# zhaowenlan1779/hekaton-system

Hardware: AMD Instinct MI355X
Metric: subcircuit Groth16 proofs/sec (whole node), big-merkle (higher is better)
Workload: dtype u32 limbs (Montgomery mod-p integers)

## Files before the change

### hekaton_system_amd/csrc/curve_ops_impl.cuh

```cuda
#pragma once
#include "msm_driver.cuh"
#include "endo.cuh"

namespace hk {

inline u32 msm_pick_c_plain(size_t n, u32 fr_bits) {
    u32 best = 4;
    double best_cost = 1e300;
    for (u32 c = 3; c <= 12; c++) {
        u32 W = (fr_bits + 2 + c - 1) / c;
        u64 NB = (u64)W << (c - 1);
        if (NB > (u64)MSM_LDS_COUNTERS) continue;
        double cost = (double)n * W + 4.0 * (double)NB;
        if (cost < best_cost) { best_cost = cost; best = c; }
    }
    return best;
}
inline u32 msm_pick_c_tables(size_t n, u32 fr_bits) {
    u32 best = 6;
    double best_cost = 1e300;
    for (u32 c = 5; c <= 16; c++) {
        u32 W = (fr_bits + 2 + c - 1) / c;
        double cost = (double)n * W + 6.0 * (double)(1u << (c - 1));
        if (cost < best_cost) { best_cost = cost; best = c; }
    }
    return best;
}

template <class C>
struct Ops final : CurveOps {
    typedef typename C::Fr Fr;
    typedef typename C::Fq Fq;
    typedef typename C::Fq2 Fq2;
    typedef VerifyRun<typename Fq::Params> Verify;
    typedef CodecRun<typename Fq::Params> Codec;

    Ops() : CurveOps(sizeof(Fr), sizeof(Fq), sizeof(Affine<Fq>), sizeof(Affine<Fq2>), sizeof(Fp12<typename Fq::Params>)) {}

    template <class F>
    struct OneMsm {
        bool small;
        const MsmPlan* p;
        u32 n;
        XYZZ<F>*xy, *tab, *res;
        Affine<F>* aff;
        SortBufs sb;
        typename MsmRun<F>::Bufs rb;

        void carve(Carve& c) {
            if (small) {
                xy = c.n<XYZZ<F>>(n);
                tab = (XYZZ<F>*)c.take(endo_tab_bytes<F>(n));
            } else {
                MsmSort<Fr>::alloc(c, *p, &sb);
                MsmRun<F>::alloc(c, *p, &rb);
            }
            res = c.n<XYZZ<F>>(1);
            aff = c.n<Affine<F>>(1);
        }
        hk_status run(hipStream_t s, const Affine<F>* bases, const void* scalars, int mont, void* out, hipMemcpyKind kind,
                      hipEvent_t ev0 = nullptr, hipEvent_t ev1 = nullptr) const {
            if (small) {
                HK_TRY(MsmRun<F>::small_msm(s, bases, scalars, mont, n, tab, xy, res));
            } else {
                HK_TRY(MsmSort<Fr>::run(s, *p, (const u32*)scalars, mont, sb));
                HK_TRY(MsmRun<F>::run(s, *p, bases, n, 0, sb, rb, res, ev0, ev1));
            }
            HK_TRY(MsmRun<F>::to_affine(s, res, aff, 1));
            HK_HIP(hipMemcpyAsync(out, aff, sizeof(Affine<F>), kind, s));
            return HK_OK;
        }
    };

    template <class F>
    static hk_status msm_plain(hk_ctx* ctx, const void* bases, size_t n_bases, const void* scalars,
                               size_t n_scalars, int mont, int checked, void* out) {
        if (checked && n_bases != n_scalars) return HK_ERR_LEN;
        size_t n = n_bases < n_scalars ? n_bases : n_scalars;
        if (n == 0) { memset(out, 0, sizeof(Affine<F>)); return HK_OK; }
        if (!bases || !scalars) return HK_ERR_ARG;
        if (n >= (1u << 26)) return HK_ERR_ARG;
        Staged in[2] = {staged(scalars, n * sizeof(Fr)), staged(bases, n * sizeof(Affine<F>))};
        LaneGuard g(ctx);
        Lane* L = g.lane;
        if (!L) return HK_ERR_DEVICE;
        const bool small = n * EndoOf<F>::K <= SPLIT_MAX_LANES && !getenv("HK_MSM_NO_SMALL");
        MsmPlan p;
        if (!small)
            p = msm_make_plan((u32)n, C::FR_BITS, msm_pick_c_plain(n, C::FR_BITS), 0xffffffffu, ctx->max_lanes0, C::Fr::Params::MOD,
                              C::Fr::Params::N);
        OneMsm<F> msm{small, &p, (u32)n};
        HK_TRY(L->carve([&](Carve& c) { stage_carve(c, in, 2); msm.carve(c); }));
        HK_TRY(stage_upload(L, in, 2));
        HK_TRY(msm.run(L->stream, (const Affine<F>*)in[1].p, in[0].p, mont, out, hipMemcpyDeviceToHost));
        return L->settle();
    }

    hk_status msm(hk_ctx* ctx, int group, const void* bases, size_t n_bases, const void* scalars,
                  size_t n_scalars, int mont, int checked, void* out) override {
        if (group == 1) return msm_plain<Fq>(ctx, bases, n_bases, scalars, n_scalars, mont, checked, out);
        return msm_plain<Fq2>(ctx, bases, n_bases, scalars, n_scalars, mont, checked, out);
    }

    size_t max_private_bytes() override {
        size_t m = MsmRun<Fq>::max_private_bytes();
        size_t b = MsmRun<Fq2>::max_private_bytes();
        if (b > m) m = b;
        b = PairRun<typename Fq::Params>::max_private_bytes();
        if (b > m) m = b;
        b = Verify::max_private_bytes();
        if (b > m) m = b;
        b = Codec::max_private_bytes();
        if (b > m) m = b;
        b = finish_private_bytes();
        return b > m ? b : m;
    }

    hk_status ntt(hk_ctx*, void*, unsigned, int, int) override;
    hk_status witness_map(hk_ctx*, const hk_csr*, const hk_csr*, const hk_csr*, size_t, size_t,
                          const void*, size_t, void*, size_t, size_t*) override;
    void ctx_release(hk_ctx*) override;
    hk_status pk_upload(hk_ctx*, const hk_pk_desc*, hk_pk**) override;
    void pk_free(hk_pk*) override;
    hk_status bases_upload(hk_ctx*, int, const void*, size_t, hk_bases**) override;
    void bases_free(hk_bases*) override;
    hk_status msm_bases(hk_ctx*, const hk_bases*, const void*, size_t, int, int, void*) override;
    hk_status fixed_base(hk_ctx*, int, const void*, const void*, size_t, int, void*) override;
    hk_status scalar_pairing(hk_ctx*, int, const void*, const void*, size_t, void*) override;
    hk_status points_lincomb(hk_ctx*, int, const void* const*, const void*, size_t, size_t, void*) override;
    template <class F>
    static hk_status points_fold(hk_ctx*, size_t, const void* const*, const void* const*, const void*, unsigned, size_t, void* const*);
    hk_status points_fold_many(hk_ctx*, int, size_t, const void* const*, const void* const*, const void*, unsigned, size_t,
                               void* const*) override;
    hk_status field_convert(hk_ctx*, int, const void*, void*, size_t, int) override;
    hk_status assignment_from_bits(hk_ctx*, const void*, size_t, const uint32_t*, const void*, size_t, void*) override;
    hk_status wprog_upload(hk_ctx*, const uint32_t*, size_t, const uint32_t*, size_t, const uint32_t*, size_t, size_t,
                           size_t, hk_wprog**) override;
    void wprog_free(hk_wprog*) override;
    hk_status wprog_run(hk_ctx*, const hk_wprog*, const uint32_t*, size_t, const uint32_t*, const void*, size_t, void*) override;
    hk_status assignment_scatter(hk_ctx*, const uint32_t*, const void*, size_t, size_t, size_t, void*) override;
    hk_status poseidon_path(hk_ctx*, const void*, size_t, const hk_poseidon_desc*, const hk_poseidon_desc*, const void*,
                            const void*, const uint32_t*, size_t, size_t, size_t, size_t, void*) override;
    hk_status pairing_products(hk_ctx*, const void* const*, size_t, const void* const*, size_t, size_t, void*) override;
    hk_status pairing_pairs(hk_ctx*, const void* const*, size_t, const void* const*, size_t, const uint32_t*, const uint32_t*, size_t,
                            size_t, void*) override;
    hk_status gt_pow(hk_ctx*, const void*, const void*, size_t, void*, int, size_t) override;
    hk_status commit(hk_ctx*, const hk_pk*, size_t, const void*, size_t, const void*, void*) override;
    hk_status commit_batch(hk_ctx*, const hk_pk*, size_t, const void*, size_t, const void*, size_t, void*) override;
    hk_status prove_batch(hk_ctx*, const hk_pk*, size_t, size_t, const ProveRow*, size_t) override;
    static size_t finish_private_bytes();
    hk_status vk_prepare(hk_ctx* ctx, const hk_vk_desc* d, hk_vk** out) override { return Verify::vk_prepare(ctx, d, out); }
    void vk_free(hk_vk* vk) override { Verify::vk_free(vk); }
    hk_status vk_alpha_beta(const hk_vk* vk, void* out) override { return Verify::vk_alpha_beta(vk, out); }
    hk_status verify_batch(hk_ctx* ctx, const hk_vk* vk, const void* a, const void* b, const void* c, const void* ds,
                           const void* inputs, size_t n, unsigned flags, const void* rand, unsigned char* verdicts) override {
        return Verify::verify_batch(ctx, vk, a, b, c, ds, inputs, n, flags, rand, verdicts);
    }
    hk_status points_check(hk_ctx* ctx, int group, const void* pts, size_t n, unsigned char* ok) override {
        return Verify::points_check(ctx, group, pts, n, ok);
    }
    hk_status qap_eval(hk_ctx*, const hk_csr*, const hk_csr*, const hk_csr*, size_t, size_t, size_t, const void*, void*,
                       void*, void*, void*, size_t*) override;
    hk_status keygen(hk_ctx*, const hk_keygen_desc*, const hk_keygen_out*, size_t*) override;
    hk_status exec_tree(hk_ctx*, const hk_exec_tree_desc*, const hk_exec_tree_out*) override;
    hk_status stage1_witness(hk_ctx*, const hk_stage1_desc*, const uint32_t*, size_t, size_t, void*) override;
    hk_status trace_sort(hk_ctx*, uint32_t, const void*, size_t, void*, uint32_t*) override;
    hk_status stage0_witness(hk_ctx*, const uint32_t*, uint32_t, uint32_t, const void*, const void*, const uint32_t*, size_t,
                             void*) override;
    hk_status r1cs_check(hk_ctx*, const hk_csr*, const hk_csr*, const hk_csr*, const void*, size_t, size_t, hk_r1cs_verdict*,
                         uint32_t*, void*, size_t) override;
    hk_status pk_r1cs_check(hk_ctx*, const hk_pk*, const void*, size_t, size_t, hk_r1cs_verdict*, uint32_t*, void*, size_t) override;
    hk_status sha_tree(hk_ctx*, const void*, uint32_t, uint32_t, uint32_t, const hk_sha_tree_out*) override;
    hk_status sha_tree_inputs(hk_ctx*, const void*, const void*, uint32_t, uint32_t, const uint32_t*, size_t, uint32_t*) override;
    hk_status ram_stage0_witness(hk_ctx*, const uint32_t*, uint32_t, uint32_t, const void*, const void*, const uint32_t*, size_t,
                                 void*) override;
    hk_status ram_stage1_witness(hk_ctx*, const hk_ram_stage1_desc*, const uint32_t*, size_t, size_t, void*) override;
    hk_status r1cs_job_trace(hk_ctx*, const hk_r1cs_job_desc*, void*) override;
    hk_status r1cs_job_witness(hk_ctx*, const hk_r1cs_job_desc*, const uint32_t*, size_t, size_t, size_t, void*) override;
    hk_status vkd_trace(hk_ctx*, const hk_vkd_desc*, void*, void*) override;
    hk_status vkd_witness(hk_ctx*, const hk_vkd_desc*, const uint32_t*, size_t, size_t, const hk_vkd_cols*, void*) override;
    hk_status vkd_tree(hk_ctx*, const hk_vkd_tree_desc*, void*, void*, uint8_t*) override;
    hk_status scalar_powers(hk_ctx*, const void*, size_t, size_t, void*) override;
    hk_status ipa_quotient(hk_ctx*, const void*, size_t, const void*, const void*, size_t, void*) override;
    hk_status class_power_sums(hk_ctx*, const void*, const uint32_t*, size_t, size_t, void*) override;
    hk_status field_sqrt(hk_ctx* ctx, int which, const void* in, size_t n, void* out, unsigned char* ok) override {
        return Codec::field_sqrt(ctx, which, in, n, out, ok);
    }
    hk_status points_decompress(hk_ctx* ctx, int group, const void* x_canon, const unsigned char* flags, size_t n, int check,
                                void* points_out, unsigned char* status) override {
        return Codec::points_decompress(ctx, group, x_canon, flags, n, check, points_out, status);
    }
    hk_status points_compress(hk_ctx* ctx, int group, const void* points, size_t n, void* x_canon_out,
                              unsigned char* flags_out) override {
        return Codec::points_compress(ctx, group, points, n, x_canon_out, flags_out);
    }
};

}
```

### hekaton_system_amd/csrc/h_basis.cuh

```cuda
#pragma once
#include "ntt_host.cuh"
#include "csr.cuh"
#include "endo.cuh"
#include "h_basis_plan.h"

namespace hk {

template <class Fr, class F>
__device__ XYZZ<F> hb_mul(const XYZZ<F>& p, const Fr& s_mont, const EndoSplit<2>& E) {
    XYZZ<F> acc = XYZZ<F>::inf();
    if (p.is_inf()) return acc;
    Fr k = Fr::from_mont(s_mont);
    u32 c[8], mag[2][6];
    HK_UNROLL for (int l = 0; l < 8; l++) c[l] = l < Fr::N ? k.v[l] : 0u;
    u32 neg = endo_decompose<2>(c, E, mag);
    XYZZ<F> t[3];
    Affine<F> q;
    q.x = p.x; q.y = p.y;
    t[0] = p;
    t[1] = p;
    t[1].x = EndoOf<F>::apply(q).x;
    if (neg & 1u) t[0].y = F::neg(p.y);
    if (neg & 2u) t[1].y = F::neg(p.y);
    t[2] = ec_add_ni(t[0], t[1]);
    HK_NOUNROLL for (int b = EndoOf<F>::STEPS - 1; b >= 0; b--) {
        u32 m = ((mag[0][b >> 5] >> (b & 31)) & 1u) | (((mag[1][b >> 5] >> (b & 31)) & 1u) << 1);
        if (m == 0 && acc.is_inf()) continue;
        acc = ec_dbl_ni(acc);
        if (m) acc = ec_add_ni(acc, t[m - 1]);
    }
    return acc;
}

template <class Fr, class F>
__global__ void __launch_bounds__(64)
k_hb_load(const Affine<F>* __restrict__ h_g, u32 h_len, u32 log_m, const Fr* __restrict__ pw_ginv, Fr c0, Fr c1,
          EndoSplit<2> E, XYZZ<F>* __restrict__ x) {
    u32 i = blockIdx.x * blockDim.x + threadIdx.x;
    if (i >> log_m) return;
    const u32 v = blockIdx.y;
    u32 r = log_m ? (__brev(i) >> (32 - log_m)) : 0u;
    XYZZ<F> o = XYZZ<F>::inf();
    if (i < h_len) {
        Fr s = v ? c1 : Fr::mul(c0, pow_from_tables(pw_ginv, i, log_m));
        o = hb_mul(XYZZ<F>::from_affine(ld_vec(&h_g[i])), s, E);
    }
    st_vec(&x[((size_t)v << log_m) + r], o);
}

template <class Fr, class F>
__global__ void __launch_bounds__(64)
k_hb_stage(XYZZ<F>* __restrict__ x, const Fr* __restrict__ tws, u32 s, u32 log_m, EndoSplit<2> E) {
    u32 t = blockIdx.x * blockDim.x + threadIdx.x;
    if (t >> (log_m - 1)) return;
    XYZZ<F>* vec = x + ((size_t)blockIdx.y << log_m);
    const u32 half = 1u << s, pos = t & (half - 1u);
    const size_t i0 = ((size_t)(t >> s) << (s + 1)) | pos, i1 = i0 + half;
    XYZZ<F> u = ld_vec(&vec[i0]), w = ld_vec(&vec[i1]);
    if (pos) w = hb_mul(w, fr_load(&tws[(half - 1u) + pos]), E);
    st_vec(&vec[i0], ec_add_ni(u, w));
    st_vec(&vec[i1], ec_add_ni(u, ec_neg(w)));
}

template <class Fr, class F>
__global__ void __launch_bounds__(64)
k_hb_ccols(const u64* __restrict__ col_ptr, const u32* __restrict__ row, const u32* __restrict__ src,
           const Fr* __restrict__ val, const Affine<F>* __restrict__ g, const u32* __restrict__ hv,
           const Affine<F>* __restrict__ heavy, const Affine<F>* __restrict__ ck_last, u32 first_last, u32 n_v,
           EndoSplit<2> E, XYZZ<F>* __restrict__ out) {
    u32 k = blockIdx.x * blockDim.x + threadIdx.x;
    if (k >= n_v) return;
    XYZZ<F> acc = XYZZ<F>::inf();
    if (hv[k]) {
        acc = XYZZ<F>::from_affine(ld_vec(&heavy[hv[k] - 1]));
    } else {
        HK_NOUNROLL for (u64 e = col_ptr[k]; e < col_ptr[k + 1]; e++)
            acc = ec_add_ni(acc, hb_mul(XYZZ<F>::from_affine(ld_vec(&g[row[e]])), fr_load(&val[src[e]]), E));
    }
    acc = ec_neg(acc);
    if (k >= first_last) acc = ec_madd_ni(acc, ld_vec(&ck_last[k - first_last]));
    st_vec(&out[k], acc);
}

template <class C>
struct HBasis {
    typedef typename C::Fr Fr;
    typedef typename C::Fq Fq;
    typedef NttHost<C> N;

    static size_t private_bytes() {
        size_t m = 0;
        for (const void* k : {(const void*)k_hb_load<Fr, Fq>, (const void*)k_hb_stage<Fr, Fq>, (const void*)k_hb_ccols<Fr, Fq>}) {
            size_t b = hk_private_bytes_of(k);
            if (b > m) m = b;
        }
        return m;
    }

    static hk_status transform(hk_ctx* ctx, NttTables* T, const Affine<Fq>* h_g, u32 h_len, u32 log_m, Affine<Fq>* hat,
                               Affine<Fq>* g) {
        const size_t m = (size_t)1 << log_m;
        LaneGuard lg(ctx);
        Lane* L = lg.lane;
        if (!L) return HK_ERR_DEVICE;
        XYZZ<Fq>* x;
        Fq* pref;
        HK_TRY(L->carve([&](Carve& c) { x = c.n<XYZZ<Fq>>(2 * m); pref = c.n<Fq>(2 * m); }));
        hipStream_t s = L->stream;
        static const EndoSplit<2> E = EndoOf<Fq>::split();
        Fr minv = N::size_inv(log_m), zinv = N::vanishing_inv_on_coset(log_m);
        Fr c1 = Fr::mul(zinv, minv), c0 = Fr::mul(c1, Fr::mul(minv, minv));
        hipLaunchKernelGGL((k_hb_load<Fr, Fq>), dim3((u32)((m + 63) / 64), 2), dim3(64), 0, s, h_g, h_len, log_m,
                           (const Fr*)T->pw_ginv, c0, c1, E, x);
        for (u32 st = 0; st < log_m; st++)
            hipLaunchKernelGGL((k_hb_stage<Fr, Fq>), dim3((u32)((m / 2 + 63) / 64), 2), dim3(64), 0, s, x, (const Fr*)T->tw_inv,
                               st, log_m, E);
        HK_HIP(hipGetLastError());
        HK_TRY(MsmRun<Fq>::batch_affine(s, x, hat, pref, (u32)m));
        HK_TRY(MsmRun<Fq>::batch_affine(s, x + m, g, pref + m, (u32)m));
        return L->settle();
    }

    static hk_status c_columns(hk_ctx* ctx, const CsrDev& Cm, size_t n_v, u32 log_m, const Affine<Fq>* g, const void* ck_last,
                               size_t n1, Affine<Fq>* out) {
        const size_t m = (size_t)1 << log_m, nnz = Cm.nnz;
        std::vector<u64> rp(Cm.n_rows + 1), col_ptr;
        std::vector<u32> cl(nnz), row, src;
        HK_HIP(hipMemcpy(rp.data(), Cm.row_ptr, 8 * rp.size(), hipMemcpyDeviceToHost));
        if (nnz) HK_HIP(hipMemcpy(cl.data(), Cm.col, 4 * nnz, hipMemcpyDeviceToHost));
        if (Cm.n_rows > m || !hb_transpose(rp.data(), cl.data(), Cm.n_rows, n_v, col_ptr, row, src)) return HK_ERR_ARG;
        const u32 thr = hb_heavy_threshold(getenv("HK_H_BASIS_HEAVY_COL"));
        std::vector<u32> hv(n_v, 0);
        std::vector<Affine<Fq>> heavy;
        for (size_t k = 0; k < n_v; k++)
            if (hb_col_is_heavy(col_ptr[k + 1] - col_ptr[k], thr)) hv[k] = 1;
        if (std::find(hv.begin(), hv.end(), 1u) != hv.end()) {
            std::vector<Fr> vals(nnz), dense(m, Fr::zero());
            HK_HIP(hipMemcpy(vals.data(), Cm.val, sizeof(Fr) * nnz, hipMemcpyDeviceToHost));
            hk_bases* bh = nullptr;
            HK_TRY(ctx->ops->bases_upload(ctx, 1, g, m, &bh));
            hk_status st = HK_OK;
            for (size_t k = 0; k < n_v && st == HK_OK; k++) {
                if (!hv[k]) continue;
                for (u64 e = col_ptr[k]; e < col_ptr[k + 1]; e++) dense[row[e]] = Fr::add(dense[row[e]], vals[src[e]]);
                Affine<Fq> pt;
                st = ctx->ops->msm_bases(ctx, bh, dense.data(), m, 1, 1, &pt);
                for (u64 e = col_ptr[k]; e < col_ptr[k + 1]; e++) dense[row[e]] = Fr::zero();
                heavy.push_back(pt);
                hv[k] = (u32)heavy.size();
            }
            ctx->ops->bases_free(bh);
            HK_TRY(st);
        }
        Staged in[6] = {staged(col_ptr.data(), 8 * col_ptr.size()), staged(row.data(), 4 * nnz), staged(src.data(), 4 * nnz),
                        staged(hv.data(), 4 * n_v), staged(heavy.data(), sizeof(Affine<Fq>) * heavy.size()),
                        staged(n1 ? ck_last : nullptr, sizeof(Affine<Fq>) * n1)};
        LaneGuard lg(ctx);
        Lane* L = lg.lane;
        if (!L) return HK_ERR_DEVICE;
        XYZZ<Fq>* xy;
        Fq* pref;
        HK_TRY(L->carve([&](Carve& c) { stage_carve(c, in, 6); xy = c.n<XYZZ<Fq>>(n_v); pref = c.n<Fq>(n_v); }));
        HK_TRY(stage_upload(L, in, 6));
        static const EndoSplit<2> E = EndoOf<Fq>::split();
        hipLaunchKernelGGL((k_hb_ccols<Fr, Fq>), dim3((u32)((n_v + 63) / 64)), dim3(64), 0, L->stream, (const u64*)in[0].p,
                           (const u32*)in[1].p, (const u32*)in[2].p, (const Fr*)Cm.val, g, (const u32*)in[3].p,
                           (const Affine<Fq>*)in[4].p, (const Affine<Fq>*)in[5].p, (u32)(n_v - n1), (u32)n_v, E, xy);
        HK_HIP(hipGetLastError());
        HK_TRY(MsmRun<Fq>::batch_affine(L->stream, xy, out, pref, (u32)n_v));
        return L->settle();
    }
};

}
```

### hekaton_system_amd/csrc/hk_core.hip

```cpp
#include <utility>
#include "hk_internal.h"
#include "job_args.h"
#include <hsa/hsa.h>
#include <hsa/hsa_ext_amd.h>
#include <atomic>

namespace hk {

static hsa_status_t scratch_limit_cb(hsa_agent_t a, void* data) {
    hsa_device_type_t type;
    if (hsa_agent_get_info(a, HSA_AGENT_INFO_DEVICE, &type) != HSA_STATUS_SUCCESS || type != HSA_DEVICE_TYPE_GPU)
        return HSA_STATUS_SUCCESS;
    uint64_t mx = 0;
    if (hsa_agent_get_info(a, (hsa_agent_info_t)HSA_AMD_AGENT_INFO_SCRATCH_LIMIT_MAX, &mx) == HSA_STATUS_SUCCESS && mx) {
        uint64_t* best = (uint64_t*)data;
        if (*best == 0 || mx < *best) *best = mx;
    }
    return HSA_STATUS_SUCCESS;
}
static uint64_t scratch_limit_bytes() {
    static const uint64_t v = [] {
        uint64_t best = 0;
        if (hsa_init() == HSA_STATUS_SUCCESS) {
            (void)hsa_iterate_agents(scratch_limit_cb, &best);
// ... 458 lines not shown
    return ctx->ops->pairing_products(ctx, lhs_g1, n_lhs, rhs_g2, n_rhs, n, gt_out);
}
hk_status hk_multi_pairing(hk_ctx* ctx, const void* g1, const void* g2, size_t n, void* gt_out) {
    if (!ctx || !gt_out || (n && (!g1 || !g2))) return HK_ERR_ARG;
    const void* l[1] = {n ? g1 : (const void*)gt_out};
    const void* r[1] = {n ? g2 : (const void*)gt_out};
    return ctx->ops->pairing_products(ctx, l, 1, r, 1, n, gt_out);
}
hk_status hk_vk_prepare(hk_ctx* ctx, const hk_vk_desc* desc, hk_vk** out) {
    if (!ctx || !desc || !out) return HK_ERR_ARG;
    return ctx->ops->vk_prepare(ctx, desc, out);
}
void hk_vk_free(hk_vk* vk) {
    if (vk) vk->ops->vk_free(vk);
}
hk_status hk_vk_alpha_beta(const hk_vk* vk, void* gt_out) {
    if (!vk || !gt_out) return HK_ERR_ARG;
    return vk->ops->vk_alpha_beta(vk, gt_out);
}
hk_status hk_verify_batch(hk_ctx* ctx, const hk_vk* vk, const void* a_g1, const void* b_g2, const void* c_g1, const void* ds_g1,
                          const void* inputs_mont, size_t n, unsigned flags, const void* rand_mont, uint8_t* verdicts) {
    if (!ctx || !vk || vk->ctx != ctx) return HK_ERR_ARG;
    return ctx->ops->verify_batch(ctx, vk, a_g1, b_g2, c_g1, ds_g1, inputs_mont, n, flags, rand_mont, verdicts);
}
hk_status hk_points_check_g1(hk_ctx* ctx, const void* points, size_t n, uint8_t* ok) {
    if (!ctx || (n && (!points || !ok))) return HK_ERR_ARG;
    return ctx->ops->points_check(ctx, 1, points, n, ok);
}
hk_status hk_points_check_g2(hk_ctx* ctx, const void* points, size_t n, uint8_t* ok) {
    if (!ctx || (n && (!points || !ok))) return HK_ERR_ARG;
    return ctx->ops->points_check(ctx, 2, points, n, ok);
}
hk_status hk_ctx_gt_bytes(const hk_ctx* ctx, size_t* gt) {
    if (!ctx || !gt) return HK_ERR_ARG;
    *gt = ctx->ops->gt_bytes;
    return HK_OK;
}
hk_status hk_field_convert(hk_ctx* ctx, int which, const void* in, void* out, size_t n, int to_mont) {
    if (!ctx || (which != 0 && which != 1) || (n && (!in || !out))) return HK_ERR_ARG;
    return ctx->ops->field_convert(ctx, which, in, out, n, to_mont);
}
hk_status hk_ntt(hk_ctx* ctx, void* data, unsigned log_m, int inverse, int coset) {
    if (!ctx || !data) return HK_ERR_ARG;
    return ctx->ops->ntt(ctx, data, log_m, inverse, coset);
}
hk_status hk_witness_map(hk_ctx* ctx, const hk_csr* A, const hk_csr* B, const hk_csr* C, size_t n_inst,
                         size_t n_constraints, const void* z_mont, size_t n_v, void* h_out,
                         size_t h_capacity, size_t* m_out) {
    if (!ctx || !A || !B || !C || !z_mont || !h_out) return HK_ERR_ARG;
    return ctx->ops->witness_map(ctx, A, B, C, n_inst, n_constraints, z_mont, n_v, h_out, h_capacity, m_out);
}
hk_status hk_pk_upload(hk_ctx* ctx, const hk_pk_desc* desc, hk_pk** out) {
    if (!ctx || !desc || !out) return HK_ERR_ARG;
    return ctx->ops->pk_upload(ctx, desc, out);
}
void hk_pk_free(hk_pk* pk) {
    if (!pk) return;
    pk->ops->pk_free(pk);
}
hk_status hk_commit(hk_ctx* ctx, const hk_pk* pk, size_t stage, const void* w, size_t n, const void* kappa,
                    void* out) {
    if (!ctx || !pk || !kappa || !out) return HK_ERR_ARG;
    return ctx->ops->commit(ctx, pk, stage, w, n, kappa, out);
}
hk_status hk_commit_batch(hk_ctx* ctx, const hk_pk* pk, size_t stage, const void* w, size_t n, const void* kappas, size_t batch,
                          void* out) {
    if (!ctx || !pk || (batch && (!kappas || !out))) return HK_ERR_ARG;
    return ctx->ops->commit_batch(ctx, pk, stage, w, n, kappas, batch, out);
}
hk_status hk_prove(hk_ctx* ctx, const hk_pk* pk, const void* z, size_t n_v, const void* r, const void* s,
                   const void* kappas, size_t n_kappas, void* a, void* b, void* c) {
    if (!ctx || !pk || !z || !r || !s || !a || !b || !c) return HK_ERR_ARG;
    HK_TRY(ctx->ops->prove_batch(ctx, pk, n_v, n_kappas, nullptr, 0));
    if (n_kappas && !kappas) return HK_ERR_ARG;
    const hk::ProveCall call = {{z, r, s, kappas, a, b, c}, n_v, n_kappas};
    if (hk::gather_trace() && hk::tl_prev_chunk_end_us)
        fprintf(stderr, "[hekaton] gather arrive gap_us=%lld\n", (long long)(hk::now_us() - hk::tl_prev_chunk_end_us));
    hk::ProveResult res = ctx->prove_q.submit(pk, call, [&](const hk_pk* key, hk::ProveCoalescer::Member* const* ms, size_t n) {
        std::vector<hk::ProveRow> rows(n);
        for (size_t i = 0; i < n; i++) rows[i] = ms[i]->item->row;
        hk_status st = ctx->ops->prove_batch(ctx, key, ms[0]->item->n_v, ms[0]->item->n_kappas, rows.data(), n);
        hk_timings t = tl_last_timings;
        const float f = 1.0f / (float)n;
        for (float* x : {&t.total_ms, &t.digits_ms, &t.msm_a_ms, &t.msm_b_g1_ms, &t.msm_b_g2_ms, &t.msm_l_ms, &t.witness_map_ms,
                         &t.msm_h_ms, &t.finish_ms, &t.accum_kernel_ms, &t.accum_h_ms, &t.keygen_qap_ms, &t.keygen_scalars_ms,
                         &t.keygen_sweeps_ms})
            *x *= f;
        if (t.accum_kernel_launches) t.accum_kernel_launches = 4;
        t.batch_proofs = (uint32_t)n;
        int64_t end_us = 0;
        if (hk::gather_trace()) {
            end_us = hk::now_us();
            fprintf(stderr, "[hekaton] gather chunk n=%zu arena_allocs=%u\n", n, hk::g_arena_allocs.load());
        }
        for (size_t i = 0; i < n; i++) ms[i]->result = hk::ProveResult{st, t, end_us};
    });
    hk::tl_prev_chunk_end_us = res.end_us;
    tl_last_timings = res.timings;
    return res.status;
}
hk_status hk_prove_batch(hk_ctx* ctx, const hk_pk* pk, const void* z, size_t n_v, const void* r, const void* s,
                         const void* kappas, size_t n_kappas, size_t batch, void* a, void* b, void* c) {
    if (!ctx || !pk) return HK_ERR_ARG;
    HK_TRY(ctx->ops->prove_batch(ctx, pk, n_v, n_kappas, nullptr, 0));
    if (batch == 0) return HK_OK;
    if (!z || !r || !s || !a || !b || !c || (n_kappas && !kappas)) return HK_ERR_ARG;
    const size_t fr = ctx->ops->fr_bytes, g1 = ctx->ops->g1_bytes, g2 = ctx->ops->g2_bytes;
    std::vector<hk::ProveRow> rows(batch);
    for (size_t i = 0; i < batch; i++)
        rows[i] = {(const char*)z + i * n_v * fr, (const char*)r + i * fr, (const char*)s + i * fr,
                   n_kappas ? (const char*)kappas + i * n_kappas * fr : nullptr, (char*)a + i * g1, (char*)b + i * g2,
                   (char*)c + i * g1};
    return ctx->ops->prove_batch(ctx, pk, n_v, n_kappas, rows.data(), batch);
}

hk_status hk_qap_eval(hk_ctx* ctx, const hk_csr* A, const hk_csr* B, const hk_csr* C, size_t n_inst, size_t n_constraints,
                      size_t n_v, const void* t, void* a, void* b, void* c, void* zt, size_t* m_out) {
    if (!ctx) return HK_ERR_ARG;
    return ctx->ops->qap_eval(ctx, A, B, C, n_inst, n_constraints, n_v, t, a, b, c, zt, m_out);
}
hk_status hk_keygen(hk_ctx* ctx, const hk_keygen_desc* desc, const hk_keygen_out* out, size_t* m_out) {
    if (!ctx || !desc || !out) return HK_ERR_ARG;
    return ctx->ops->keygen(ctx, desc, out, m_out);
}
hk_status hk_exec_tree(hk_ctx* ctx, const hk_exec_tree_desc* desc, const hk_exec_tree_out* out) {
    if (!ctx || !desc || !out) return HK_ERR_ARG;
    return ctx->ops->exec_tree(ctx, desc, out);
}
hk_status hk_stage1_witness(hk_ctx* ctx, const hk_stage1_desc* desc, const uint32_t* sub_index, size_t batch, size_t n_v,
                            void* z_out) {
    if (!ctx || !desc) return HK_ERR_ARG;
    return ctx->ops->stage1_witness(ctx, desc, sub_index, batch, n_v, z_out);
}
hk_status hk_trace_sort(hk_ctx* ctx, uint32_t entry_fields, const void* time_entries_mont, size_t n_entries,
                        void* addr_entries_mont_out, uint32_t* perm_out) {
    if (!ctx) return HK_ERR_ARG;
    return ctx->ops->trace_sort(ctx, entry_fields, time_entries_mont, n_entries, addr_entries_mont_out, perm_out);
}
hk_status hk_stage0_witness(hk_ctx* ctx, const uint32_t* offsets, uint32_t n_sub, uint32_t n_portals, const void* time_entries_mont,
                            const void* addr_entries_mont, const uint32_t* sub_index, size_t batch, void* w_out) {
    if (!ctx) return HK_ERR_ARG;
    return ctx->ops->stage0_witness(ctx, offsets, n_sub, n_portals, time_entries_mont, addr_entries_mont, sub_index, batch, w_out);
}
hk_status hk_r1cs_check(hk_ctx* ctx, const hk_csr* A, const hk_csr* B, const hk_csr* C, const void* z_mont, size_t n_v, size_t batch,
                        hk_r1cs_verdict* verdicts, uint32_t* bad_rows, void* bad_vals, size_t cap) {
    if (!ctx || !A || !B || !C) return HK_ERR_ARG;
    return ctx->ops->r1cs_check(ctx, A, B, C, z_mont, n_v, batch, verdicts, bad_rows, bad_vals, cap);
}
hk_status hk_pk_r1cs_check(hk_ctx* ctx, const hk_pk* pk, const void* z_mont, size_t n_v, size_t batch, hk_r1cs_verdict* verdicts,
                           uint32_t* bad_rows, void* bad_vals, size_t cap) {
    if (!ctx || !pk) return HK_ERR_ARG;
    return ctx->ops->pk_r1cs_check(ctx, pk, z_mont, n_v, batch, verdicts, bad_rows, bad_vals, cap);
}
hk_status hk_sha_tree(hk_ctx* ctx, const void* leaves, uint32_t n_sub, uint32_t ns, uint32_t n_portals, const hk_sha_tree_out* out) {
    if (!ctx || !leaves || !out) return HK_ERR_ARG;
    return ctx->ops->sha_tree(ctx, leaves, n_sub, ns, n_portals, out);
}
hk_status hk_sha_tree_inputs(hk_ctx* ctx, const void* leaves, const void* digests, uint32_t n_sub, uint32_t n_inputs,
                             const uint32_t* sub_index, size_t batch, uint32_t* inputs_out) {
    if (!ctx) return HK_ERR_ARG;
    return ctx->ops->sha_tree_inputs(ctx, leaves, digests, n_sub, n_inputs, sub_index, batch, inputs_out);
}
hk_status hk_ram_stage0_witness(hk_ctx* ctx, const uint32_t* offsets, uint32_t n_sub, uint32_t n_portals,
                                const void* time_entries_mont, const void* addr_entries_mont, const uint32_t* sub_index, size_t batch,
                                void* w_out) {
    if (!ctx) return HK_ERR_ARG;
    return ctx->ops->ram_stage0_witness(ctx, offsets, n_sub, n_portals, time_entries_mont, addr_entries_mont, sub_index, batch, w_out);
}
hk_status hk_ram_stage1_witness(hk_ctx* ctx, const hk_ram_stage1_desc* desc, const uint32_t* sub_index, size_t batch, size_t n_v,
                                void* z_out) {
    if (!ctx || !desc) return HK_ERR_ARG;
    return ctx->ops->ram_stage1_witness(ctx, desc, sub_index, batch, n_v, z_out);
}
hk_status hk_r1cs_job_trace(hk_ctx* ctx, const hk_r1cs_job_desc* desc, void* time_entries_mont_out) {
    if (!ctx || !desc) return HK_ERR_ARG;
    return ctx->ops->r1cs_job_trace(ctx, desc, time_entries_mont_out);
}
hk_status hk_r1cs_job_witness(hk_ctx* ctx, const hk_r1cs_job_desc* desc, const uint32_t* sub_index, size_t batch, size_t n_v,
                              size_t body_col0, void* z_out) {
    if (!ctx || !desc) return HK_ERR_ARG;
    return ctx->ops->r1cs_job_witness(ctx, desc, sub_index, batch, n_v, body_col0, z_out);
}
hk_status hk_vkd_trace(hk_ctx* ctx, const hk_vkd_desc* desc, void* values_mont_out, void* time_entries_mont_out) {
    if (!ctx || !desc) return HK_ERR_ARG;
    return ctx->ops->vkd_trace(ctx, desc, values_mont_out, time_entries_mont_out);
}
hk_status hk_vkd_witness(hk_ctx* ctx, const hk_vkd_desc* desc, const uint32_t* sub_index, size_t batch, size_t n_v,
                         const hk_vkd_cols* cols, void* z_out) {
    if (!ctx || !desc) return HK_ERR_ARG;
    return ctx->ops->vkd_witness(ctx, desc, sub_index, batch, n_v, cols, z_out);
}
hk_status hk_vkd_tree(hk_ctx* ctx, const hk_vkd_tree_desc* desc, void* siblings_mont_out, void* roots_mont_out, uint8_t* status_out) {
    if (!ctx || !desc) return HK_ERR_ARG;
    return ctx->ops->vkd_tree(ctx, desc, siblings_mont_out, roots_mont_out, status_out);
}
hk_status hk_scalar_powers(hk_ctx* ctx, const void* x_mont, size_t n, size_t reps, void* out) {
    if (!ctx) return HK_ERR_ARG;
    return ctx->ops->scalar_powers(ctx, x_mont, n, reps, out);
}
hk_status hk_ipa_quotient(hk_ctx* ctx, const void* challenges_mont, size_t l, const void* rho_mont, const void* z_mont,
                          size_t shift, void* q_out) {
    if (!ctx) return HK_ERR_ARG;
    return ctx->ops->ipa_quotient(ctx, challenges_mont, l, rho_mont, z_mont, shift, q_out);
}
hk_status hk_class_power_sums(hk_ctx* ctx, const void* x_mont, const uint32_t* class_of, size_t n, size_t n_classes,
                              void* sums_out) {
    if (!ctx) return HK_ERR_ARG;
    return ctx->ops->class_power_sums(ctx, x_mont, class_of, n, n_classes, sums_out);
}

static bool codec_bufs_bad(const void* const* in, const size_t* in_len, int n_in, const void* const* out, const size_t* out_len,
                           int n_out) {
    for (int a = 0; a < n_in; a++)
        if (!in[a]) return true;
    for (int b = 0; b < n_out; b++) {
        if (!out[b]) return true;
        for (int a = 0; a < n_in; a++)
            if (hk::bufs_overlap(in[a], in_len[a], out[b], out_len[b])) return true;
        for (int c = 0; c < b; c++)
            if (hk::bufs_overlap(out[c], out_len[c], out[b], out_len[b])) return true;
    }
    return false;
}
hk_status hk_field_sqrt(hk_ctx* ctx, int which, const void* in_mont, size_t n, void* out_mont, uint8_t* ok) {
    if (!ctx || (which != 1 && which != 2) || n >= ((size_t)1 << 31)) return HK_ERR_ARG;
    if (n == 0) return HK_OK;
    const size_t eb = ctx->ops->fq_bytes * (size_t)which;
    const void* in[1] = {in_mont};
    const void* out[2] = {out_mont, ok};
    const size_t il[1] = {n * eb}, ol[2] = {n * eb, n};
    if (codec_bufs_bad(in, il, 1, out, ol, 2)) return HK_ERR_ARG;
    return ctx->ops->field_sqrt(ctx, which, in_mont, n, out_mont, ok);
}
static hk_status points_decompress(hk_ctx* ctx, int group, const void* x_canon, const uint8_t* flags, size_t n, int check,
                                   void* points_out, uint8_t* status) {
    if (!ctx || n >= ((size_t)1 << 31)) return HK_ERR_ARG;
    if (n == 0) return HK_OK;
    const size_t xb = ctx->ops->fq_bytes * (size_t)group;
    const void* in[2] = {x_canon, flags};
    const void* out[2] = {points_out, status};
    const size_t il[2] = {n * xb, n}, ol[2] = {2 * n * xb, n};
    if (codec_bufs_bad(in, il, 2, out, ol, 2)) return HK_ERR_ARG;
    return ctx->ops->points_decompress(ctx, group, x_canon, flags, n, check, points_out, status);
}
static hk_status points_compress(hk_ctx* ctx, int group, const void* points, size_t n, void* x_canon_out, uint8_t* flags_out) {
    if (!ctx || n >= ((size_t)1 << 31)) return HK_ERR_ARG;
    if (n == 0) return HK_OK;
    const size_t xb = ctx->ops->fq_bytes * (size_t)group;
    const void* in[1] = {points};
    const void* out[2] = {x_canon_out, flags_out};
    const size_t il[1] = {2 * n * xb}, ol[2] = {n * xb, n};
    if (codec_bufs_bad(in, il, 1, out, ol, 2)) return HK_ERR_ARG;
    return ctx->ops->points_compress(ctx, group, points, n, x_canon_out, flags_out);
}
hk_status hk_points_decompress_g1(hk_ctx* ctx, const void* x_canon, const uint8_t* flags, size_t n, int check, void* points_out,
                                  uint8_t* status) {
    return points_decompress(ctx, 1, x_canon, flags, n, check, points_out, status);
}
hk_status hk_points_decompress_g2(hk_ctx* ctx, const void* x_canon, const uint8_t* flags, size_t n, int check, void* points_out,
                                  uint8_t* status) {
    return points_decompress(ctx, 2, x_canon, flags, n, check, points_out, status);
}
hk_status hk_points_compress_g1(hk_ctx* ctx, const void* points, size_t n, void* x_canon_out, uint8_t* flags_out) {
    return points_compress(ctx, 1, points, n, x_canon_out, flags_out);
}
hk_status hk_points_compress_g2(hk_ctx* ctx, const void* points, size_t n, void* x_canon_out, uint8_t* flags_out) {
    return points_compress(ctx, 2, points, n, x_canon_out, flags_out);
}

}

extern "C" void hk_keccak_f1600(uint64_t* st) {
    static const uint64_t RC[24] = {
        0x0000000000000001ull, 0x0000000000008082ull, 0x800000000000808aull, 0x8000000080008000ull, 0x000000000000808bull,
        0x0000000080000001ull, 0x8000000080008081ull, 0x8000000000008009ull, 0x000000000000008aull, 0x0000000000000088ull,
        0x0000000080008009ull, 0x000000008000000aull, 0x000000008000808bull, 0x800000000000008bull, 0x8000000000008089ull,
        0x8000000000008003ull, 0x8000000000008002ull, 0x8000000000000080ull, 0x000000000000800aull, 0x800000008000000aull,
        0x8000000080008081ull, 0x8000000000008080ull, 0x0000000080000001ull, 0x8000000080008008ull};
    static const int ROT[5][5] = {{0, 36, 3, 41, 18}, {1, 44, 10, 45, 2}, {62, 6, 43, 15, 61}, {28, 55, 25, 21, 56}, {27, 20, 39, 8, 14}};
    auto rol = [](uint64_t x, int n) { return n ? (x << n) | (x >> (64 - n)) : x; };
    for (int rnd = 0; rnd < 24; rnd++) {
        uint64_t c[5], d[5], b[25];
        for (int x = 0; x < 5; x++) c[x] = st[x] ^ st[x + 5] ^ st[x + 10] ^ st[x + 15] ^ st[x + 20];
        for (int x = 0; x < 5; x++) d[x] = c[(x + 4) % 5] ^ rol(c[(x + 1) % 5], 1);
        for (int i = 0; i < 25; i++) st[i] ^= d[i % 5];
        for (int x = 0; x < 5; x++)
            for (int y = 0; y < 5; y++) b[y + 5 * ((2 * x + 3 * y) % 5)] = rol(st[x + 5 * y], ROT[x][y]);
        for (int y = 0; y < 5; y++)
            for (int x = 0; x < 5; x++) st[x + 5 * y] = b[x + 5 * y] ^ (~b[(x + 1) % 5 + 5 * y] & b[(x + 2) % 5 + 5 * y]);
        st[0] ^= RC[rnd];
    }
}
```

### hekaton_system_amd/csrc/hk_internal.h

```cpp
#pragma once
#include <hip/hip_runtime.h>
#include <condition_variable>
#include <cstdio>
#include <cstring>
#include <map>
#include <mutex>
#include <string>
#include <vector>

#include "../../include/hekaton.h"
#include "coalesce.h"
#include "msm.cuh"
#include "stream_plan.h"

#define HK_HIP(expr)                                                                         \
    do {                                                                                     \
        hipError_t _e = (expr);                                                              \
        if (_e != hipSuccess) {                                                              \
            fprintf(stderr, "[hekaton] HIP error %s at %s:%d: %s\n", hipGetErrorName(_e),    \
                    __FILE__, __LINE__, #expr);                                              \
            return HK_ERR_DEVICE;                                                            \
        }                                                                                    \
    } while (0)

#define HK_TRY(expr)                       \
    do {                                   \
        hk_status _s = (expr);             \
        if (_s != HK_OK) return _s;        \
    } while (0)

namespace hk {

struct CurveBn254 {
    typedef Fp<Bn254FrP> Fr;
    typedef Fp<Bn254FqP> Fq;
    typedef Fp2<Bn254FqP> Fq2;
    static constexpr u32 FR_BITS = HK_BN254_FR_BITS;
    static constexpr u32 TWO_ADICITY = HK_BN254_TWO_ADICITY;
    static constexpr u32 ROOT[8] = HK_BN254_FR_ROOT;
    static constexpr u32 GEN[8] = HK_BN254_FR_GEN;
    static constexpr u32 GEN_INV[8] = HK_BN254_FR_GEN_INV;
};
struct CurveBls381 {
    typedef Fp<Bls381FrP> Fr;
    typedef Fp<Bls381FqP> Fq;
    typedef Fp2<Bls381FqP> Fq2;
    static constexpr u32 FR_BITS = HK_BLS12_381_FR_BITS;
    static constexpr u32 TWO_ADICITY = HK_BLS12_381_TWO_ADICITY;
    static constexpr u32 ROOT[8] = HK_BLS12_381_FR_ROOT;
    static constexpr u32 GEN[8] = HK_BLS12_381_FR_GEN;
    static constexpr u32 GEN_INV[8] = HK_BLS12_381_FR_GEN_INV;
};

template <class F> struct ScalarOf;
template <> struct ScalarOf<CurveBn254::Fq> { typedef CurveBn254::Fr type; };
template <> struct ScalarOf<CurveBn254::Fq2> { typedef CurveBn254::Fr type; };
template <> struct ScalarOf<CurveBls381::Fq> { typedef CurveBls381::Fr type; };
template <> struct ScalarOf<CurveBls381::Fq2> { typedef CurveBls381::Fr type; };

struct Carve {
    char* base = nullptr;
    size_t off = 0;
    void* take(size_t bytes) {
        size_t o = (off + 255) & ~(size_t)255;
        off = o + bytes;
        return base ? base + o : nullptr;
    }
    template <class T> T* n(size_t count) { return (T*)take(count * sizeof(T)); }
};

struct Lane {
    hipStream_t stream = nullptr;
    char* arena = nullptr;
    size_t arena_cap = 0;
    hipEvent_t ev[32];
    hipStream_t side[PROVE_MAX_STREAMS - 1] = {};
    unsigned n_streams = 1;
    bool prove = false;
    bool busy = false;
    bool settled = false;
    hk_timings timings;
    std::vector<void*> retired;
    hk_ctx* owner = nullptr;

    hk_status reserve(size_t bytes);
    template <class Fn> hk_status carve(Fn&& fn) {
        Carve count;
        fn(count);
        HK_TRY(reserve(count.off));
        Carve real;
        real.base = arena;
        fn(real);
        if (real.off != count.off) {
            fprintf(stderr, "[hekaton] scratch carve is not deterministic (%zu bytes counted, %zu carved)\n", count.off, real.off);
            return HK_ERR_DEVICE;
        }
        settled = false;
        return HK_OK;
    }
    hipStream_t stream_at(unsigned i) const { return i ? side[i - 1] : stream; }
    hk_status settle() {
        for (unsigned i = 0; i < n_streams; i++) HK_HIP(hipStreamSynchronize(stream_at(i)));
        settled = true;
        return HK_OK;
    }
};

struct NttTables;

struct ProveRow {
    const void* z;
    const void* r;
    const void* s;
    const void* kappas;
    void *a, *b, *c;
};

struct ProveResult {
    hk_status status;
    hk_timings timings;
    int64_t end_us;
};

enum { PROVE_GATHER_US = 1000 };

struct ProveCall {
    ProveRow row;
    size_t n_v, n_kappas;
};

enum { PROVE_COALESCE_RUNNING = 2 };
typedef Coalescer<const hk_pk*, ProveCall, ProveResult> ProveCoalescer;

}

namespace hk {
struct CurveOps {
    const size_t fr_bytes, fq_bytes, g1_bytes, g2_bytes, gt_bytes;

    virtual hk_status msm(hk_ctx*, int group, const void* bases, size_t n_bases, const void* scalars,
                          size_t n_scalars, int mont, int checked, void* out) = 0;
    virtual size_t max_private_bytes() = 0;
    virtual hk_status ntt(hk_ctx*, void* data, unsigned log_m, int inverse, int coset) = 0;
    virtual hk_status witness_map(hk_ctx*, const hk_csr* A, const hk_csr* B, const hk_csr* C, size_t n_inst,
                                  size_t n_c, const void* z, size_t n_v, void* h_out, size_t h_cap, size_t* m_out) = 0;
    virtual void ctx_release(hk_ctx*) = 0;
    virtual hk_status pk_upload(hk_ctx*, const hk_pk_desc*, hk_pk**) = 0;
    virtual void pk_free(hk_pk*) = 0;
    virtual hk_status bases_upload(hk_ctx*, int group, const void* bases, size_t n, hk_bases** out) = 0;
    virtual void bases_free(hk_bases*) = 0;
    virtual hk_status msm_bases(hk_ctx*, const hk_bases*, const void* scalars, size_t n_scalars, int mont, int checked,
                                void* out) = 0;
    virtual hk_status fixed_base(hk_ctx*, int group, const void* base, const void* scalars, size_t n, int mont,
                                 void* out) = 0;
    virtual hk_status scalar_pairing(hk_ctx*, int group, const void* points, const void* scalars, size_t n, void* out) = 0;
    virtual hk_status points_lincomb(hk_ctx*, int group, const void* const* vecs, const void* coeffs, size_t k, size_t n,
                                     void* out) = 0;
    virtual hk_status points_fold_many(hk_ctx*, int group, size_t k, const void* const* lo, const void* const* hi,
                                       const void* coeffs, unsigned neg_mask, size_t n, void* const* out) = 0;
    virtual hk_status field_convert(hk_ctx*, int which, const void* in, void* out, size_t n, int to_mont) = 0;
    virtual hk_status assignment_from_bits(hk_ctx*, const void* bits, size_t n_v, const uint32_t* full_cols,
                                           const void* full_vals, size_t n_full, void* z_out) = 0;
    virtual hk_status wprog_upload(hk_ctx*, const uint32_t* ops, size_t n_ops, const uint32_t* refs, size_t n_refs,
                                   const uint32_t* map, size_t n_v, size_t n_values, size_t n_inputs, hk_wprog** out) = 0;
    virtual void wprog_free(hk_wprog*) = 0;
    virtual hk_status wprog_run(hk_ctx*, const hk_wprog*, const uint32_t* inputs, size_t batch, const uint32_t* full_cols,
                                const void* full_vals, size_t n_full, void* z_out) = 0;
    virtual hk_status assignment_scatter(hk_ctx*, const uint32_t* full_cols, const void* full_vals, size_t n_full, size_t batch,
                                         size_t n_v, void* z_out) = 0;
    virtual hk_status poseidon_path(hk_ctx*, const void* consts, size_t n_consts, const hk_poseidon_desc* leaf_hash,
                                    const hk_poseidon_desc* node_hash, const void* leaf, const void* siblings,
                                    const uint32_t* index, size_t depth, size_t batch, size_t n_v, size_t col0, void* z_out) = 0;
    virtual hk_status pairing_products(hk_ctx*, const void* const* lhs, size_t n_lhs, const void* const* rhs, size_t n_rhs,
                                       size_t n, void* out) = 0;
    virtual hk_status pairing_pairs(hk_ctx*, const void* const* lhs, size_t n_lhs, const void* const* rhs, size_t n_rhs,
                                    const uint32_t* pair_lhs, const uint32_t* pair_rhs, size_t n_pairs, size_t n, void* out) = 0;
    virtual hk_status gt_pow(hk_ctx*, const void* gt_in, const void* scalars, size_t n, void* gt_out, int in_gt,
                             size_t group_len) = 0;
    virtual hk_status commit(hk_ctx*, const hk_pk*, size_t stage, const void* w, size_t n, const void* kappa,
                             void* out) = 0;
    virtual hk_status commit_batch(hk_ctx*, const hk_pk*, size_t stage, const void* w, size_t n, const void* kappas, size_t batch,
                                   void* out) = 0;
    virtual hk_status prove_batch(hk_ctx*, const hk_pk*, size_t n_v, size_t n_kappas, const ProveRow* rows, size_t batch) = 0;
    virtual hk_status vk_prepare(hk_ctx*, const hk_vk_desc*, hk_vk**) = 0;
    virtual void vk_free(hk_vk*) = 0;
    virtual hk_status vk_alpha_beta(const hk_vk*, void*) = 0;
    virtual hk_status verify_batch(hk_ctx*, const hk_vk*, const void* a, const void* b, const void* c, const void* ds,
                                   const void* inputs, size_t n, unsigned flags, const void* rand, unsigned char* verdicts) = 0;
    virtual hk_status points_check(hk_ctx*, int group, const void* pts, size_t n, unsigned char* ok) = 0;
    virtual hk_status qap_eval(hk_ctx*, const hk_csr* A, const hk_csr* B, const hk_csr* C, size_t n_inst, size_t n_c, size_t n_v,
                               const void* t, void* a, void* b, void* c, void* zt, size_t* m_out) = 0;
    virtual hk_status keygen(hk_ctx*, const hk_keygen_desc*, const hk_keygen_out*, size_t* m_out) = 0;
    virtual hk_status exec_tree(hk_ctx*, const hk_exec_tree_desc*, const hk_exec_tree_out*) = 0;
    virtual hk_status stage1_witness(hk_ctx*, const hk_stage1_desc*, const uint32_t* sub_index, size_t batch, size_t n_v,
                                     void* z_out) = 0;
    virtual hk_status trace_sort(hk_ctx*, uint32_t entry_fields, const void* time_entries, size_t n_entries, void* addr_entries_out,
                                 uint32_t* perm_out) = 0;
    virtual hk_status stage0_witness(hk_ctx*, const uint32_t* offsets, uint32_t n_sub, uint32_t n_portals, const void* time_entries,
                                     const void* addr_entries, const uint32_t* sub_index, size_t batch, void* w_out) = 0;
    virtual hk_status r1cs_check(hk_ctx*, const hk_csr* A, const hk_csr* B, const hk_csr* C, const void* z, size_t n_v, size_t batch,
                                 hk_r1cs_verdict* verdicts, uint32_t* bad_rows, void* bad_vals, size_t cap) = 0;
    virtual hk_status pk_r1cs_check(hk_ctx*, const hk_pk*, const void* z, size_t n_v, size_t batch, hk_r1cs_verdict* verdicts,
                                    uint32_t* bad_rows, void* bad_vals, size_t cap) = 0;
    virtual hk_status sha_tree(hk_ctx*, const void* leaves, uint32_t n_sub, uint32_t ns, uint32_t n_portals,
                               const hk_sha_tree_out* out) = 0;
    virtual hk_status sha_tree_inputs(hk_ctx*, const void* leaves, const void* digests, uint32_t n_sub, uint32_t n_inputs,
                                      const uint32_t* sub_index, size_t batch, uint32_t* inputs_out) = 0;

    virtual hk_status ram_stage0_witness(hk_ctx*, const uint32_t* offsets, uint32_t n_sub, uint32_t n_portals,
                                         const void* time_entries, const void* addr_entries, const uint32_t* sub_index,
                                         size_t batch, void* w_out) = 0;
    virtual hk_status ram_stage1_witness(hk_ctx*, const hk_ram_stage1_desc*, const uint32_t* sub_index, size_t batch, size_t n_v,
                                         void* z_out) = 0;
    virtual hk_status r1cs_job_trace(hk_ctx*, const hk_r1cs_job_desc*, void* time_entries_out) = 0;
    virtual hk_status r1cs_job_witness(hk_ctx*, const hk_r1cs_job_desc*, const uint32_t* sub_index, size_t batch, size_t n_v,
                                       size_t body_col0, void* z_out) = 0;
    virtual hk_status vkd_trace(hk_ctx*, const hk_vkd_desc*, void* values_out, void* time_entries_out) = 0;
    virtual hk_status vkd_witness(hk_ctx*, const hk_vkd_desc*, const uint32_t* sub_index, size_t batch, size_t n_v,
                                  const hk_vkd_cols* cols, void* z_out) = 0;
    virtual hk_status vkd_tree(hk_ctx*, const hk_vkd_tree_desc*, void* siblings_out, void* roots_out, uint8_t* status_out) = 0;
    virtual hk_status scalar_powers(hk_ctx*, const void* x, size_t n, size_t reps, void* out) = 0;
    virtual hk_status ipa_quotient(hk_ctx*, const void* challenges, size_t l, const void* rho, const void* z, size_t shift,
                                   void* q_out) = 0;
    virtual hk_status class_power_sums(hk_ctx*, const void* x, const uint32_t* class_of, size_t n, size_t n_classes,
                                       void* sums_out) = 0;
    virtual hk_status field_sqrt(hk_ctx*, int which, const void* in, size_t n, void* out, unsigned char* ok) = 0;
    virtual hk_status points_decompress(hk_ctx*, int group, const void* x_canon, const unsigned char* flags, size_t n, int check,
                                        void* points_out, unsigned char* status) = 0;
    virtual hk_status points_compress(hk_ctx*, int group, const void* points, size_t n, void* x_canon_out,
                                      unsigned char* flags_out) = 0;

protected:
    CurveOps(size_t fr, size_t fq, size_t g1, size_t g2, size_t gt)
        : fr_bytes(fr), fq_bytes(fq), g1_bytes(g1), g2_bytes(g2), gt_bytes(gt) {}
    ~CurveOps() = default;
};
CurveOps* curve_ops_bn254();
CurveOps* curve_ops_bls381();
}

struct hk_ctx {
    hk_curve curve;
    hk::CurveOps* ops = nullptr;
    int device;
    int profiling = 0;
    std::mutex mu;
    std::condition_variable cv;
    std::vector<hk::Lane*> lanes;
    size_t max_lanes = 8;
    std::vector<hk::Lane*> prove_lanes;
    unsigned prove_streams = 1;
    std::condition_variable prove_cv;
    hk::NttTables* ntt = nullptr;
    hk_timings last;
    uint32_t max_lanes0 = 262144;
    void* presize_kernel = nullptr;
    struct FbTable { int group; std::string base; void* table; bool ready; };
    enum { FB_CACHE_MAX = 8 };
    std::vector<FbTable> fb_cache;
    hk::ProveCoalescer prove_q;
    explicit hk_ctx(long gather_us)
        : prove_q(hk::PROVE_COALESCE_RUNNING, HK_PROVE_BATCH_CHUNK, hk::ProveResult{HK_ERR_NOMEM, {}, 0}, gather_us) {}
};

struct hk_pk {
    hk::CurveOps* ops;
    hk_ctx* ctx;
    void* impl;
};

struct hk_vk {
    hk::CurveOps* ops;
    hk_ctx* ctx;
    void* impl;
};

struct hk_bases {
    hk::CurveOps* ops;
    hk_ctx* ctx;
    void* impl;
};

namespace hk {
struct WprogImpl {
    uint32_t *ops = nullptr, *refs = nullptr, *map = nullptr;
    uint32_t n_ops = 0, n_refs = 0, n_values = 0, n_inputs = 0;
    size_t n_v = 0;
};
}
struct hk_wprog {
    hk::CurveOps* ops;
    hk_ctx* ctx;
    hk::WprogImpl* impl;
};

namespace hk {

struct ProveLaneTag {};
struct LaneGuard {
    hk_ctx* ctx;
    Lane* lane;
    LaneGuard(hk_ctx* c);
    LaneGuard(hk_ctx* c, ProveLaneTag);
    ~LaneGuard();
};

bool is_device_ptr(const void* p);
static inline hipMemcpyKind h2d_kind(const void* src) {
    return is_device_ptr(src) ? hipMemcpyDeviceToDevice : hipMemcpyHostToDevice;
}
static inline float ev_ms(hipEvent_t a, hipEvent_t b) {
    float ms = 0.f;
    if (hipEventElapsedTime(&ms, a, b) != hipSuccess) { (void)hipGetLastError(); return 0.f; }
    return ms;
}

struct Staged {
    const void* buf;
    size_t bytes;
    size_t scratch;
    void* p;
};
static inline Staged staged(const void* buf, size_t bytes) {
    return {buf, bytes, buf && !is_device_ptr(buf) ? bytes : 0, nullptr};
}
static inline void stage_carve(Carve& c, Staged* s, size_t n) {
    for (size_t k = 0; k < n; k++) {
        void* slice = c.take(s[k].scratch);
        s[k].p = s[k].scratch ? slice : (void*)s[k].buf;
    }
}
static inline hk_status stage_upload(Lane* L, const Staged* s, size_t n) {
    for (size_t k = 0; k < n; k++)
        if (s[k].scratch) HK_HIP(hipMemcpyAsync(s[k].p, s[k].buf, s[k].bytes, hipMemcpyHostToDevice, L->stream));
    return HK_OK;
}
static inline hk_status stage_download(Lane* L, const Staged* s, size_t n) {
    for (size_t k = 0; k < n; k++)
        if (s[k].scratch) HK_HIP(hipMemcpyAsync((void*)s[k].buf, s[k].p, s[k].bytes, hipMemcpyDeviceToHost, L->stream));
    return HK_OK;
}

}
```

### hekaton_system_amd/csrc/msm.cuh

```cuda
#pragma once
#include <cstdlib>
#include "ec.cuh"

namespace hk {

constexpr int MSM_MAX_LEVELS = 16;
#ifndef HK_MSM_LVL_L
#define HK_MSM_LVL_L 16
#endif
constexpr u32 MSM_LVL_L = HK_MSM_LVL_L;
constexpr int MSM_TAIL_THREADS = 256;
constexpr int MSM_WSUM_THREADS = 256;
#ifndef HK_MSM_SORT_THREADS
#define HK_MSM_SORT_THREADS 1024
#endif
constexpr int MSM_SORT_THREADS = HK_MSM_SORT_THREADS;
constexpr int MSM_ENTRY_GROUP_SHIFT = 26;
constexpr int MSM_LDS_COUNTERS = 32768;
constexpr u32 MSM_RANK_NONE = 0xffffffffu;

struct MsmPlan {
    u32 n;
    u32 c;
    u32 B;
    u32 W;
    u32 WP;
    u32 F;
    u32 NB;
    u32 n_levels;
    u32 T[MSM_MAX_LEVELS];
    u32 Lmin0;
    u32 gshift;
    u32 chunk;
    u32 K;
    u32 kconst[10];
};

struct LevelInfo { u32 count, L, active; };
HK_HD LevelInfo msm_level_info(const MsmPlan& p, u32 E, int k) {
    LevelInfo li;
    li.count = E;
    u32 L = (E + p.T[0] - 1) / p.T[0];
    if (L < p.Lmin0) L = p.Lmin0;
    li.L = L;
    li.active = (E + L - 1) / L;
    for (int j = 1; j <= k; j++) {
        li.count = 2 * li.active;
        li.L = MSM_LVL_L;
        li.active = (li.count + li.L - 1) / li.L;
    }
    return li;
}

HK_HD size_t msm_sorted_stride(const MsmPlan& p) { return (size_t)p.n * p.W + 1; }
HK_HD size_t msm_digits_stride(const MsmPlan& p) { return (size_t)p.n * p.W + 8; }
HK_HD size_t msm_p1_stride(const MsmPlan& p) { return p.n_levels > 1 ? 2ull * p.T[1] : 2ull; }

#if defined(__HIPCC__)

template <class Fr>
__device__ __forceinline__ void msm_load_scalar(const u32* scalars, size_t i, int is_mont,
                                                const MsmPlan& p, u32 (&sp)[10]) {
    Fr s;
    const uint4* src = reinterpret_cast<const uint4*>(scalars + i * Fr::N);
#pragma unroll
    for (int k = 0; k < Fr::N / 4; k++) {
        uint4 v = src[k];
        s.v[4 * k] = v.x; s.v[4 * k + 1] = v.y; s.v[4 * k + 2] = v.z; s.v[4 * k + 3] = v.w;
    }
    if (is_mont) s = Fr::from_mont(s);
    u64 carry = 0;
#pragma unroll
    for (int k = 0; k < Fr::N; k++) {
        carry += (u64)s.v[k] + p.kconst[k];
        sp[k] = (u32)carry;
        carry >>= 32;
    }
    carry += p.kconst[Fr::N];
    sp[Fr::N] = (u32)carry;
    sp[Fr::N + 1] = 0;
}

template <u32 C>
__device__ __forceinline__ int msm_digit_at(const u32 (&sp)[10], u32 w) {
    const u32 o = C * w;
    const u32 limb = o >> 5, sh = o & 31;
    u32 e = sp[limb] >> sh;
    if (sh + C > 32) e |= sp[limb + 1] << (32 - sh);
    return (int)(e & ((1u << C) - 1u)) - (int)(1u << (C - 1));
}

template <class Fr, u32 C>
__device__ __forceinline__ void msm_hist_scalar(const u32 (&sp)[10], size_t i, const MsmPlan& p, short* __restrict__ digits,
                                                u32* h) {
    constexpr u32 WMAX = (Fr::N * 32 + 2 + C - 1) / C;
#pragma unroll
    for (u32 w = 0; w < WMAX; w++) {
        if (w >= p.W) break;
        int d = msm_digit_at<C>(sp, w);
        digits[(size_t)w * p.n + i] = (short)d;
        if (d != 0) {
            u32 mag = d < 0 ? (u32)(-d) : (u32)d;
            atomicAdd(&h[(p.WP == 1 ? 0u : w % p.WP) * p.B + mag - 1], 1u);
        }
    }
}

template <class Fr>
__global__ void __launch_bounds__(MSM_SORT_THREADS)
k_msm_hist(const u32* __restrict__ scalars_all, size_t scalar_stride_words, int is_mont, MsmPlan p,
           u32* __restrict__ count_all, short* __restrict__ digits_all) {
    const size_t pr = blockIdx.y;
    const u32* __restrict__ scalars = scalars_all + pr * scalar_stride_words;
    u32* __restrict__ count = count_all + pr * p.NB;
    short* __restrict__ digits = digits_all + pr * msm_digits_stride(p);
    __shared__ u32 h[MSM_LDS_COUNTERS];
    for (u32 b = threadIdx.x; b < p.NB; b += blockDim.x) h[b] = 0;
    __syncthreads();
    size_t base = (size_t)blockIdx.x * p.chunk;
    for (u32 k = threadIdx.x; k < p.chunk; k += blockDim.x) {
        size_t i = base + k;
        if (i >= p.n) break;
        u32 sp[10];
        msm_load_scalar<Fr>(scalars, i, is_mont, p, sp);
        switch (p.c) {
#define HK_HIST_C(C) case C: msm_hist_scalar<Fr, C>(sp, i, p, digits, h); break;
            HK_HIST_C(3) HK_HIST_C(4) HK_HIST_C(5) HK_HIST_C(6) HK_HIST_C(7) HK_HIST_C(8) HK_HIST_C(9) HK_HIST_C(10)
            HK_HIST_C(11) HK_HIST_C(12) HK_HIST_C(13) HK_HIST_C(14) HK_HIST_C(15) HK_HIST_C(16)
#undef HK_HIST_C
        }
    }
    __syncthreads();
    for (u32 b = threadIdx.x; b < p.NB; b += blockDim.x) {
        u32 v = h[b];
        if (v) atomicAdd(&count[b], v);
    }
}

template <int UNUSED>
__global__ void __launch_bounds__(1024)
k_msm_scan(const u32* __restrict__ count_all, u32* __restrict__ start_all, u32* __restrict__ cursor_all, u32 NB) {
    const size_t pr = blockIdx.x;
    const u32* __restrict__ count = count_all + pr * NB;
    u32* __restrict__ start = start_all + pr * (NB + 1);
    u32* __restrict__ cursor = cursor_all + pr * NB;
    __shared__ u32 part[1024];
    u32 per = (NB + 1023) / 1024;
    u32 lo = threadIdx.x * per, hi = min(lo + per, NB);
    u32 s = 0;
    for (u32 b = lo; b < hi; b++) s += count[b];
    part[threadIdx.x] = s;
    __syncthreads();
    for (u32 off = 1; off < 1024; off <<= 1) {
        u32 v = threadIdx.x >= off ? part[threadIdx.x - off] : 0;
        __syncthreads();
        part[threadIdx.x] += v;
        __syncthreads();
    }
    u32 run = threadIdx.x ? part[threadIdx.x - 1] : 0;
    for (u32 b = lo; b < hi; b++) {
        start[b] = run;
        cursor[b] = run;
        run += count[b];
    }
    if (threadIdx.x == 1023) start[NB] = part[1023];
}

__device__ __forceinline__ u32 msm_mag(int d) { return d < 0 ? (u32)(-d) : (u32)d; }
template <class Fr>
__global__ void __launch_bounds__(MSM_SORT_THREADS)
k_msm_scatter(const short* __restrict__ digits_all, MsmPlan p, u32* __restrict__ cursor_all, u32* __restrict__ sorted_all) {
    const size_t pr = blockIdx.y;
    const short* __restrict__ digits = digits_all + pr * msm_digits_stride(p);
    u32* __restrict__ cursor = cursor_all + pr * p.NB;
    u32* __restrict__ sorted = sorted_all + pr * msm_sorted_stride(p);
    __shared__ u32 h[MSM_LDS_COUNTERS];
    for (u32 b = threadIdx.x; b < p.NB; b += blockDim.x) h[b] = 0;
    __syncthreads();
    size_t base = (size_t)blockIdx.x * p.chunk;
    for (u32 k = threadIdx.x; k < p.chunk; k += blockDim.x) {
        size_t i = base + k;
        if (i >= p.n) break;
        for (u32 w = 0; w < p.W; w++) {
            int d = digits[(size_t)w * p.n + i];
            if (d != 0) atomicAdd(&h[(w % p.WP) * p.B + msm_mag(d) - 1], 1u);
        }
    }
    __syncthreads();
    for (u32 b = threadIdx.x; b < p.NB; b += blockDim.x) {
        u32 v = h[b];
        if (v) h[b] = atomicAdd(&cursor[b], v);
    }
    __syncthreads();
    for (u32 k = threadIdx.x; k < p.chunk; k += blockDim.x) {
        size_t i = base + k;
        if (i >= p.n) break;
        for (u32 w = 0; w < p.W; w++) {
            int d = digits[(size_t)w * p.n + i];
            if (d != 0) {
                u32 pos = atomicAdd(&h[(w % p.WP) * p.B + msm_mag(d) - 1], 1u);
                sorted[pos] = ((w / p.WP) << p.gshift) | (u32)i | (d < 0 ? 0x80000000u : 0u);
            }
        }
    }
}

constexpr u32 MSM_SUB_TILE = 1024;
constexpr u32 MSM_SUB_WORDS = MSM_SUB_TILE / 64;
constexpr int MSM_SUB_THREADS = 256;
HK_HD u32 msm_sub_tiles(const MsmPlan& src) { return (u32)(((u64)src.n * src.W) / MSM_SUB_TILE) + 1u; }

template <int UNUSED>
__global__ void __launch_bounds__(MSM_SUB_THREADS)
k_msm_sub_mark(const u32* __restrict__ sorted_all, const u32* __restrict__ start_all, MsmPlan ps,
               const u32* __restrict__ rank, u64* __restrict__ mask_all, u32* __restrict__ tcount_all) {
    const size_t pr = blockIdx.y;
    const u32 tiles = msm_sub_tiles(ps);
    const u32 tile = blockIdx.x * (MSM_SUB_THREADS / 64) + (threadIdx.x >> 6), lane = threadIdx.x & 63;
    if (tile >= tiles) return;
    const u32* __restrict__ sorted = sorted_all + pr * msm_sorted_stride(ps);
    const u32 E = start_all[pr * (ps.NB + 1) + ps.NB];
    u64* __restrict__ mask = mask_all + (pr * tiles + tile) * MSM_SUB_WORDS;
    const u32 imask = (1u << ps.gshift) - 1u;
    u32 kept = 0;
#pragma unroll 4
    for (u32 k = 0; k < MSM_SUB_WORDS; k++) {
        const u32 pos = tile * MSM_SUB_TILE + k * 64 + lane;
        bool keep = false;
        if (pos < E) keep = rank[sorted[pos] & imask] != MSM_RANK_NONE;
        const u64 word = __ballot(keep);
        if (lane == 0) mask[k] = word;
        kept += (u32)__popcll(word);
    }
    if (lane == 0) tcount_all[pr * tiles + tile] = kept;
}

template <int UNUSED>
__global__ void __launch_bounds__(MSM_SUB_THREADS)
k_msm_sub_emit(const u32* __restrict__ sorted_all, MsmPlan ps, const u32* __restrict__ rank,
               const u64* __restrict__ mask_all, const u32* __restrict__ toff_all, MsmPlan pd, u32* __restrict__ out_all) {
    const size_t pr = blockIdx.y;
    const u32 tiles = msm_sub_tiles(ps);
    const u32 tile = blockIdx.x * (MSM_SUB_THREADS / 64) + (threadIdx.x >> 6), lane = threadIdx.x & 63;
    if (tile >= tiles) return;
    const u32* __restrict__ sorted = sorted_all + pr * msm_sorted_stride(ps);
    u32* __restrict__ out = out_all + pr * msm_sorted_stride(pd);
    const u64* __restrict__ mask = mask_all + (pr * tiles + tile) * MSM_SUB_WORDS;
    const u32 imask = (1u << ps.gshift) - 1u;
    const u64 below = ((u64)1 << lane) - 1u;
    u32 run = toff_all[pr * tiles + tile] - toff_all[pr * tiles];
#pragma unroll 4
    for (u32 k = 0; k < MSM_SUB_WORDS; k++) {
        const u64 word = mask[k];
        if ((word >> lane) & 1u) {
            const u32 e = sorted[tile * MSM_SUB_TILE + k * 64 + lane];
            const u32 g = (e & 0x7fffffffu) >> ps.gshift;
            out[run + (u32)__popcll(word & below)] = (e & 0x80000000u) | (g << pd.gshift) | rank[e & imask];
        }
        run += (u32)__popcll(word);
    }
}

template <int UNUSED>
__global__ void __launch_bounds__(256)
k_msm_sub_starts(const u32* __restrict__ start_src_all, MsmPlan ps, const u64* __restrict__ mask_all,
                 const u32* __restrict__ toff_all, u32* __restrict__ start_dst_all) {
    const size_t pr = blockIdx.y;
    const u32 b = blockIdx.x * blockDim.x + threadIdx.x;
    if (b > ps.NB) return;
    const u32 tiles = msm_sub_tiles(ps);
    const u32 pos = start_src_all[pr * (ps.NB + 1) + b];
    const u32 tile = pos / MSM_SUB_TILE, in = pos % MSM_SUB_TILE;
    const u64* __restrict__ mask = mask_all + (pr * tiles + tile) * MSM_SUB_WORDS;
    u32 v = toff_all[pr * tiles + tile] - toff_all[pr * tiles];
    for (u32 k = 0; k < in / 64; k++) v += (u32)__popcll(mask[k]);
    if (in % 64) v += (u32)__popcll(mask[in / 64] & (((u64)1 << (in % 64)) - 1u));
    start_dst_all[pr * (ps.NB + 1) + b] = v;
}

template <class T>
__device__ __forceinline__ T ld_vec(const T* p) {
    static_assert(sizeof(T) % 16 == 0, "16-byte multiples");
    T r;
    const uint4* s = reinterpret_cast<const uint4*>(p);
    uint4* d = reinterpret_cast<uint4*>(&r);
#pragma unroll
    for (int k = 0; k < (int)(sizeof(T) / 16); k++) d[k] = s[k];
    return r;
}
// ... 455 lines not shown
```

### hekaton_system_amd/csrc/msm_driver.cuh

```cuda
#pragma once
#include "hk_internal.h"
#include "pairing.cuh"

namespace hk {

static inline size_t hk_private_bytes_of(const void* kernel) {
    hipFuncAttributes fa;
    if (hipFuncGetAttributes(&fa, kernel) != hipSuccess) { (void)hipGetLastError(); return 0; }
    return (size_t)fa.localSizeBytes;
}

struct SortBufs {
    u32* count;
    u32* start;
    u32* cursor;
    u32* sorted;
    short* digits;
    u64* mask = nullptr;
    u32* tcount = nullptr;
    u32* toff = nullptr;
    u32* tops = nullptr;
};

template <class Fr>
struct MsmSort {
    static void alloc(Carve& c, const MsmPlan& p, SortBufs* out, u32 batch = 1);
    static void alloc_sub(Carve& c, const MsmPlan& src, const MsmPlan& p, SortBufs* out, u32 batch = 1);
    static hk_status sublist(hipStream_t s, const MsmPlan& src, const SortBufs& sb_src, const MsmPlan& dst, const u32* rank,
                             const SortBufs& sb_dst, u32 batch = 1);
    static hk_status run(hipStream_t s, const MsmPlan& p, const u32* scalars_d, int is_mont,
                         const SortBufs& sb, bool count_is_zero = false, u32 batch = 1, size_t scalar_stride = 0);
};

template <class F>
struct MsmRun {
    struct Bufs {
        XYZZ<F>* buckets;
        u32* pkeys[2];
        XYZZ<F>* ppts[2];
        XYZZ<F>* red;
        XYZZ<F>* wsum;
    };
    static void alloc(Carve& c, const MsmPlan& p, Bufs* out, u32 batch = 1);
    static hk_status run(hipStream_t s, const MsmPlan& p, const Affine<F>* table, u32 n_bases, u32 idx_off,
                         const SortBufs& sb, const Bufs& b, XYZZ<F>* result_d,
                         hipEvent_t ev0, hipEvent_t ev1, u32 batch = 1, u32 res_stride = 1);
    static hk_status build_tables(hipStream_t s, Affine<F>* table, u32 n, u32 groups, u32 shift_bits);
    static hk_status to_affine(hipStream_t s, const XYZZ<F>* in, Affine<F>* out, u32 n);
    static hk_status fixed_base(hipStream_t s, const Affine<F>* base, const void* scalars, int is_mont,
                                u32 n, Affine<F>* table, XYZZ<F>* xy, F* pref, Affine<F>* out, bool build_table = true);
    static hk_status batch_affine(hipStream_t s, const XYZZ<F>* in, Affine<F>* out, F* pref, u32 n);
    static hk_status scalar_mul_each(hipStream_t s, const Affine<F>* pts, const void* scalars_mont, u32 n,
                                     XYZZ<F>* xy, F* pref, Affine<F>* out, XYZZ<F>* tab = nullptr);
    static hk_status lincomb(hipStream_t s, const Affine<F>* const* vecs, const void* coeffs_mont, u32 k, u32 n,
                             XYZZ<F>* xy, F* pref, Affine<F>* out);
    static hk_status fold_endo(hipStream_t s, u32 k, const Affine<F>* const* lo, const Affine<F>* const* hi, const void* coeffs_mont,
                               u32 neg_mask, u32 n, XYZZ<F>* tab, XYZZ<F>* xy, F* pref, Affine<F>* out, bool long_mags = false);
    static hk_status small_msm(hipStream_t s, const Affine<F>* bases, const void* scalars, int mont, u32 n, XYZZ<F>* tab,
                               XYZZ<F>* xy, XYZZ<F>* result);
    static hk_status small_msm_rows(hipStream_t s, const Affine<F>* bases, const void* scalars, u32 seg, u32 batch, XYZZ<F>* tab,
                                    XYZZ<F>* xy, XYZZ<F>* result);
    static size_t max_private_bytes();
};

constexpr int PAIR_LIST_MAX = 64;
struct PairList {
    u32 n;
    unsigned char a[PAIR_LIST_MAX], b[PAIR_LIST_MAX];
};

template <class P>
struct PairRun {
    static hk_status run(hipStream_t s, const Affine<Fp<P>>* g1, const Affine<Fp2<P>>* g2, u32 n, u32 n_l, u32 n_r,
                         Fp12<P>* miller, Fp12<P>* prod, Fp12<P>* out, const PairList* pairs = nullptr);
    static size_t scratch_bytes(u32 n, u32 count, u32 n_r);
    static size_t max_private_bytes();
    static u32 steps();
    static hk_status gt_pow(hipStream_t s, const Fp12<P>* in, const void* scalars_mont, u32 n, Fp12<P>* out, bool in_gt);
    static hk_status gt_prod(hipStream_t s, const Fp12<P>* in, u32 len, u32 groups, Fp12<P>* out);
};

template <class P>
struct VerifyRun {
    static hk_status vk_prepare(hk_ctx*, const hk_vk_desc*, hk_vk**);
    static void vk_free(hk_vk*);
    static hk_status vk_alpha_beta(const hk_vk*, void* gt_out);
    static hk_status verify_batch(hk_ctx*, const hk_vk*, const void* a, const void* b, const void* c, const void* ds,
                                  const void* inputs, size_t n, unsigned flags, const void* rand, unsigned char* verdicts);
    static hk_status points_check(hk_ctx*, int group, const void* pts, size_t n, unsigned char* ok);
    static size_t max_private_bytes();
};

template <class P>
struct CodecRun {
    static hk_status field_sqrt(hk_ctx*, int which, const void* in, size_t n, void* out, unsigned char* ok);
    static hk_status points_decompress(hk_ctx*, int group, const void* x_canon, const unsigned char* flags, size_t n, int check,
                                       void* points_out, unsigned char* status);
    static hk_status points_compress(hk_ctx*, int group, const void* points, size_t n, void* x_canon_out, unsigned char* flags_out);
    static size_t max_private_bytes();
};

}
```

### hekaton_system_amd/csrc/msm_driver_impl.cuh

```cuda
#pragma once
#include <hip/hip_ext.h>
#include "msm_driver.cuh"
#include "fixed_base.cuh"
#include "endo.cuh"
#include "scan.cuh"

namespace hk {

static inline bool hk_dbg_sync() { static const bool on = getenv("HK_DEBUG_SYNC") != nullptr; return on; }
#define HK_DBG(stream, name)                                                              \
    do {                                                                                  \
        if (hk_dbg_sync()) {                                                              \
            fprintf(stderr, "[hk] launched %s\n", name); fflush(stderr);                  \
            hipError_t _e = hipStreamSynchronize(stream);                                 \
            fprintf(stderr, "[hk] finished %s: %s\n", name, hipGetErrorName(_e)); fflush(stderr); \
        }                                                                                 \
    } while (0)

template <class Fr>
void MsmSort<Fr>::alloc(Carve& c, const MsmPlan& p, SortBufs* out, u32 batch) {
    out->count = c.n<u32>((size_t)p.NB * batch);
    out->start = c.n<u32>((size_t)(p.NB + 1) * batch);
    out->cursor = c.n<u32>((size_t)p.NB * batch);
    out->sorted = c.n<u32>(msm_sorted_stride(p) * batch);
    out->digits = c.n<short>(msm_digits_stride(p) * batch);
}

template <class Fr>
void MsmSort<Fr>::alloc_sub(Carve& c, const MsmPlan& src, const MsmPlan& p, SortBufs* out, u32 batch) {
    const size_t tiles = (size_t)msm_sub_tiles(src) * batch;
    out->count = nullptr;
    out->cursor = nullptr;
    out->digits = nullptr;
    out->start = c.n<u32>((size_t)(p.NB + 1) * batch);
    out->sorted = c.n<u32>(msm_sorted_stride(p) * batch);
    out->mask = c.n<u64>(tiles * MSM_SUB_WORDS);
    out->tcount = c.n<u32>(tiles);
    out->toff = c.n<u32>(tiles);
    out->tops = c.n<u32>(scan_u32_tops_len(tiles));
}

template <class Fr>
hk_status MsmSort<Fr>::sublist(hipStream_t s, const MsmPlan& src, const SortBufs& sb_src, const MsmPlan& dst, const u32* rank,
                               const SortBufs& sb_dst, u32 batch) {
    if (batch == 0 || batch > 65535u) return HK_ERR_ARG;
    if (dst.c != src.c || dst.W != src.W || dst.WP != src.WP || dst.NB != src.NB || dst.n > src.n) return HK_ERR_ARG;
    const u32 tiles = msm_sub_tiles(src);
    if ((u64)tiles * batch > 0xffffffffull) return HK_ERR_ARG;
    const dim3 gt((tiles + MSM_SUB_THREADS / 64 - 1) / (MSM_SUB_THREADS / 64), batch);
    hipLaunchKernelGGL((k_msm_sub_mark<0>), gt, dim3(MSM_SUB_THREADS), 0, s, (const u32*)sb_src.sorted,
                       (const u32*)sb_src.start, src, rank, sb_dst.mask, sb_dst.tcount);
    HK_DBG(s, "k_msm_sub_mark");
    HK_TRY(scan_u32(s, sb_dst.tcount, sb_dst.toff, sb_dst.tops, tiles * batch));
    hipLaunchKernelGGL((k_msm_sub_emit<0>), gt, dim3(MSM_SUB_THREADS), 0, s, (const u32*)sb_src.sorted, src, rank,
                       (const u64*)sb_dst.mask, (const u32*)sb_dst.toff, dst, sb_dst.sorted);
    HK_DBG(s, "k_msm_sub_emit");
    hipLaunchKernelGGL((k_msm_sub_starts<0>), dim3((src.NB + 1 + 255) / 256, batch), dim3(256), 0, s,
                       (const u32*)sb_src.start, src, (const u64*)sb_dst.mask, (const u32*)sb_dst.toff, sb_dst.start);
    HK_DBG(s, "k_msm_sub_starts");
    HK_HIP(hipGetLastError());
    return HK_OK;
}

template <class Fr>
hk_status MsmSort<Fr>::run(hipStream_t s, const MsmPlan& p, const u32* scalars_d, int is_mont,
                           const SortBufs& sb, bool count_is_zero, u32 batch, size_t scalar_stride) {
    if (p.NB > (u32)MSM_LDS_COUNTERS || p.c < 3 || p.c > 16) return HK_ERR_ARG;
    if (batch == 0 || batch > 65535u) return HK_ERR_ARG;
    if (!count_is_zero) HK_HIP(hipMemsetAsync(sb.count, 0, sizeof(u32) * p.NB * batch, s));
    u32 blocks = (p.n + p.chunk - 1) / p.chunk;
    if (blocks == 0) blocks = 1;
    const size_t words = scalar_stride * (sizeof(Fr) / sizeof(u32));
    hipLaunchKernelGGL((k_msm_hist<Fr>), dim3(blocks, batch), dim3(MSM_SORT_THREADS), 0, s,
                       scalars_d, words, is_mont, p, sb.count, sb.digits);
    HK_DBG(s, "k_msm_hist");
    hipLaunchKernelGGL((k_msm_scan<0>), dim3(batch), dim3(1024), 0, s, sb.count, sb.start, sb.cursor, p.NB);
    HK_DBG(s, "k_msm_scan");
    hipLaunchKernelGGL((k_msm_scatter<Fr>), dim3(blocks, batch), dim3(MSM_SORT_THREADS), 0, s,
                       (const short*)sb.digits, p, sb.cursor, sb.sorted);
    HK_DBG(s, "k_msm_scatter");
    HK_HIP(hipGetLastError());
    return HK_OK;
}

template <class F>
static inline MsmPlan msm_lane_plan(const MsmPlan& p0, u32 batch = 1) {
    MsmPlan p = p0;
    u32 lanes = (u32)AccumOcc<F>::waves * 65536u / (batch ? batch : 1u);
    msm_set_lanes(p, lanes ? lanes : 1u);
    return p;
}

template <class F>
void MsmRun<F>::alloc(Carve& c, const MsmPlan& p0, Bufs* out, u32 batch) {
    const MsmPlan p = msm_lane_plan<F>(p0, batch);
    const size_t n0 = 2ull * p.T[0], n1 = msm_p1_stride(p);
    out->buckets = c.n<XYZZ<F>>((size_t)(p.NB + 1) * batch);
    out->pkeys[0] = c.n<u32>(n0 * batch);
    out->ppts[0] = c.n<XYZZ<F>>(n0 * batch);
    out->pkeys[1] = c.n<u32>(n1 * batch);
    out->ppts[1] = c.n<XYZZ<F>>(n1 * batch);
    out->red = c.n<XYZZ<F>>((size_t)p.WP * (p.B / p.K) * batch);
    out->wsum = c.n<XYZZ<F>>((size_t)p.WP * batch);
}

template <class F>
hk_status MsmRun<F>::run(hipStream_t s, const MsmPlan& p0, const Affine<F>* table, u32 n_bases, u32 idx_off,
                         const SortBufs& sb, const Bufs& b, XYZZ<F>* result_d,
                         hipEvent_t ev0, hipEvent_t ev1, u32 batch, u32 res_stride) {
    if (batch == 0 || batch > 65535u) return HK_ERR_ARG;
    const MsmPlan p = msm_lane_plan<F>(p0, batch);
    const size_t n0 = 2ull * p.T[0], n1 = msm_p1_stride(p);
    dim3 g0((p.T[0] + 63) / 64, batch);
    if (ev0 && ev1)
        hipExtLaunchKernelGGL((k_msm_accum0<F>), g0, dim3(64), 0, s, ev0, ev1, 0,
                              table, n_bases, idx_off, sb.sorted, sb.start, p, b.buckets, b.pkeys[0], b.ppts[0]);
    else
        hipLaunchKernelGGL((k_msm_accum0<F>), g0, dim3(64), 0, s,
                           table, n_bases, idx_off, sb.sorted, sb.start, p, b.buckets, b.pkeys[0], b.ppts[0]);
    HK_DBG(s, "k_msm_accum0");
    u32 k = 1;
    for (; k < p.n_levels && p.T[k] > (u32)MSM_TAIL_THREADS; k++) {
        int in = (k - 1) & 1, out = k & 1;
        hipLaunchKernelGGL((k_msm_accum_lvl<F>), dim3((p.T[k] + 63) / 64, batch), dim3(64), 0, s,
                           (int)k, b.pkeys[in], b.ppts[in], in ? n1 : n0, sb.start, p, b.buckets, b.pkeys[out], b.ppts[out],
                           out ? n1 : n0);
        HK_DBG(s, "k_msm_accum_lvl");
    }
    if (k < p.n_levels) {
        hipLaunchKernelGGL((k_msm_accum_tail<F>), dim3(batch), dim3(MSM_TAIL_THREADS), 0, s, (int)k, b.pkeys[0], b.ppts[0],
                           b.pkeys[1], b.ppts[1], sb.start, p, b.buckets);
        HK_DBG(s, "k_msm_accum_tail");
    }
    u32 J = p.B / p.K;
    if (p.WP == 1) {
        u32 blocks = (J + MSM_REDUCE_THREADS - 1) / MSM_REDUCE_THREADS;
        hipLaunchKernelGGL((k_msm_reduce_fused<F>), dim3(blocks, batch), dim3(MSM_REDUCE_THREADS), 0, s, b.buckets, sb.start, p,
                           b.red, result_d, res_stride);
        HK_DBG(s, "k_msm_reduce_fused");
    } else {
        const size_t rs = (size_t)p.WP * J;
        for (u32 pr = 0; pr < batch; pr++) {
            const XYZZ<F>* bk = b.buckets + (size_t)pr * (p.NB + 1);
            const u32* st = sb.start + (size_t)pr * (p.NB + 1);
            hipLaunchKernelGGL((k_msm_bucket_reduce<F>), dim3((p.WP * J + 63) / 64), dim3(64), 0, s, bk, st, p, b.red + pr * rs);
            HK_DBG(s, "k_msm_bucket_reduce");
            hipLaunchKernelGGL((k_msm_window_sum<F>), dim3(p.WP), dim3(MSM_WSUM_THREADS), 0, s, b.red + pr * rs, p,
                               b.wsum + (size_t)pr * p.WP);
            HK_DBG(s, "k_msm_window_sum");
            hipLaunchKernelGGL((k_msm_final<F>), dim3(1), dim3(64), 0, s, b.wsum + (size_t)pr * p.WP, p,
                               result_d + (size_t)pr * res_stride);
            HK_DBG(s, "k_msm_final");
        }
    }
    HK_HIP(hipGetLastError());
    return HK_OK;
}


template <class F>
size_t MsmRun<F>::max_private_bytes() {
    typedef typename ScalarOf<F>::type Fr;
    const void* ks[] = {(const void*)k_msm_accum0<F>, (const void*)k_msm_accum_lvl<F>, (const void*)k_msm_accum_tail<F>,
                        (const void*)k_msm_reduce_fused<F>, (const void*)k_msm_bucket_reduce<F>,
                        (const void*)k_msm_window_sum<F>, (const void*)k_msm_final<F>, (const void*)k_to_affine<F>,
                        (const void*)k_msm_build_tables<F>, (const void*)k_batch_affine<F>, (const void*)k_fb_table<F>,
                        (const void*)k_fb_mul<Fr, F>, (const void*)k_scalar_mul_each<Fr, F>, (const void*)k_scalar_mul_endo<Fr, F>, (const void*)k_points_fold_endo<Fr, F>, (const void*)k_points_mul_split<Fr, F, true>, (const void*)k_points_mul_split<Fr, F, false>, (const void*)k_points_sum<F>, (const void*)k_points_sum_seg<F>,
                        (const void*)k_points_lincomb<Fr, F>};
    size_t m = 0;
    for (const void* k : ks) { size_t b = hk_private_bytes_of(k); if (b > m) m = b; }
    return m;
}

template <class F>
hk_status MsmRun<F>::build_tables(hipStream_t s, Affine<F>* table, u32 n, u32 groups, u32 shift_bits) {
    if (groups <= 1 || n == 0) return HK_OK;
    hipLaunchKernelGGL((k_msm_build_tables<F>), dim3((n + 63) / 64), dim3(64), 0, s, table, n, groups,
                       shift_bits);
    HK_HIP(hipGetLastError());
    return HK_OK;
}

template <class F>
hk_status MsmRun<F>::to_affine(hipStream_t s, const XYZZ<F>* in, Affine<F>* out, u32 n) {
    hipLaunchKernelGGL((k_to_affine<F>), dim3((n + 63) / 64), dim3(64), 0, s, in, out, n);
    HK_DBG(s, "k_to_affine");
    HK_HIP(hipGetLastError());
    return HK_OK;
}

template <class F>
hk_status MsmRun<F>::batch_affine(hipStream_t s, const XYZZ<F>* in, Affine<F>* out, F* pref, u32 n) {
    if (n == 0) return HK_OK;
    u32 chunk = (n + 65535) / 65536;
    if (chunk > (u32)FB_CHUNK) chunk = FB_CHUNK;
    u32 lanes = (n + chunk - 1) / chunk;
    hipLaunchKernelGGL((k_batch_affine<F>), dim3((lanes + 63) / 64), dim3(64), 0, s, in, out, pref, n, chunk);
    HK_HIP(hipGetLastError());
    return HK_OK;
}

template <class Fr, class P, bool UNIFORM>
static inline void launch_mul_split(hipStream_t s, const SplitVecs<Fp2<P>>& v, u32 k, const Fr* scalars, u32 neg_mask, u32 n,
                                    const EndoSplit<4>& E, Jac<Fp2<P>>* tab, XYZZ<Fp2<P>>* xy, int scalars_mont = 1) {
    const bool no_quad = getenv("HK_ENDO_NO_QUAD") != nullptr;
    u32 lanes = n * 4;
    if (!no_quad && (size_t)lanes * 4 <= SPLIT_MAX_LANES) {
        typedef Fp2Q<P> Q;
        SplitVecs<Q> vq;
        for (int y = 0; y < FOLD_MAX; y++) { vq.lo[y] = (const Affine<Q>*)v.lo[y]; vq.pts[y] = (const Affine<Q>*)v.pts[y]; }
        vq.pts_mod = v.pts_mod;
        hipLaunchKernelGGL((k_points_mul_split<Fr, Q, UNIFORM>), dim3((lanes * 4 + 63) / 64, k), dim3(64), 0, s, vq, scalars,
                           neg_mask, n, E, (Jac<Q>*)tab, (XYZZ<Q>*)xy, scalars_mont);
    } else {
        hipLaunchKernelGGL((k_points_mul_split<Fr, Fp2<P>, UNIFORM>), dim3((lanes + 63) / 64, k), dim3(64), 0, s, v, scalars,
                           neg_mask, n, E, tab, xy, scalars_mont);
    }
}
template <class Fr, class P, bool UNIFORM>
static inline void launch_mul_split(hipStream_t s, const SplitVecs<Fp<P>>& v, u32 k, const Fr* scalars, u32 neg_mask, u32 n,
                                    const EndoSplit<2>& E, Jac<Fp<P>>* tab, XYZZ<Fp<P>>* xy, int scalars_mont = 1) {
    hipLaunchKernelGGL((k_points_mul_split<Fr, Fp<P>, UNIFORM>), dim3((n * 2 + 63) / 64, k), dim3(64), 0, s, v, scalars,
                       neg_mask, n, E, tab, xy, scalars_mont);
}

template <class F>
hk_status MsmRun<F>::scalar_mul_each(hipStream_t s, const Affine<F>* pts, const void* scalars_mont, u32 n,
// ... 100 lines not shown
```

### hekaton_system_amd/csrc/ntt.cuh

```cuda
#pragma once
#include "field.cuh"

namespace hk {

constexpr int NTT_TILE_LOG = 11;
constexpr int NTT_THREADS = 512;
constexpr int POW_TABLE_BITS = 11;
constexpr int POW_TABLE_SIZE = 1 << POW_TABLE_BITS;

#if defined(__HIPCC__)

template <class Fr>
__device__ __forceinline__ Fr fr_load(const Fr* p) {
    Fr r;
    const uint4* s = reinterpret_cast<const uint4*>(p);
    uint4 a = s[0], b = s[1];
    r.v[0] = a.x; r.v[1] = a.y; r.v[2] = a.z; r.v[3] = a.w;
    r.v[4] = b.x; r.v[5] = b.y; r.v[6] = b.z; r.v[7] = b.w;
    return r;
}
template <class Fr>
__device__ __forceinline__ void fr_store(Fr* p, const Fr& lazy) {
    Fr r = Fr::canon(lazy);
    uint4* d = reinterpret_cast<uint4*>(p);
    d[0] = make_uint4(r.v[0], r.v[1], r.v[2], r.v[3]);
    d[1] = make_uint4(r.v[4], r.v[5], r.v[6], r.v[7]);
}

template <class Fr>
__global__ void k_pow_table(Fr* __restrict__ tw, const Fr* __restrict__ sq, u32 count, u32 nbits) {
    u32 i = blockIdx.x * blockDim.x + threadIdx.x;
    if (i >= count) return;
    Fr acc = Fr::one();
    for (u32 k = 0; k < nbits; k++)
        if ((i >> k) & 1) acc = Fr::mul(acc, fr_load(&sq[k]));
    fr_store(&tw[i], acc);
}

template <class Fr>
__device__ __forceinline__ Fr pow_from_tables(const Fr* __restrict__ pw, u32 j, u32 logn) {
    Fr g = fr_load(&pw[j & (POW_TABLE_SIZE - 1)]);
    if (logn > POW_TABLE_BITS) g = Fr::mul(g, fr_load(&pw[POW_TABLE_SIZE + ((j >> POW_TABLE_BITS) & (POW_TABLE_SIZE - 1))]));
    if (logn > 2 * POW_TABLE_BITS) g = Fr::mul(g, fr_load(&pw[2 * POW_TABLE_SIZE + (j >> (2 * POW_TABLE_BITS))]));
    return g;
}

template <class Fr>
__global__ void k_stage_tables(Fr* __restrict__ tws, const Fr* __restrict__ tw, u32 log_table) {
    size_t i = (size_t)blockIdx.x * blockDim.x + threadIdx.x;
    if ((i + 1) >> log_table) return;
    u32 s = 31 - __clz((u32)(i + 1));
    size_t j = i + 1 - ((size_t)1 << s);
    fr_store(&tws[i], fr_load(&tw[j << (log_table - s - 1)]));
}

template <class Fr, int DIT>
__global__ void __launch_bounds__(NTT_THREADS)
k_ntt_pass4(Fr* __restrict__ data, size_t stride_vec, const Fr* __restrict__ tws, u32 logn, u32 lo, u32 nst,
            u32 cols_bits, int post, u32 npost, Fr scale, const Fr* __restrict__ pw, const Fr* __restrict__ sub,
            Fr kc) {
    extern __shared__ uint4 lds_raw[];
    Fr* lds = reinterpret_cast<Fr*>(lds_raw);
    const u32 nthr = blockDim.x;
    if (blockIdx.y >= npost) post = 0;
    Fr* vec = data + (size_t)blockIdx.y * stride_vec;
    const u32 cols = 1u << cols_bits;
    const u32 tile_elems = 1u << (nst + cols_bits);
    const u32 mid_bits = lo - cols_bits;
    const u32 mid = blockIdx.x & ((1u << mid_bits) - 1u);
    const size_t base = ((size_t)(blockIdx.x >> mid_bits) << (lo + nst)) | ((size_t)mid << cols_bits);
    for (u32 e = threadIdx.x; e < tile_elems; e += nthr) {
        u32 r = e >> cols_bits, c = e & (cols - 1);
        lds[e] = fr_load(&vec[base | ((size_t)r << lo) | c]);
    }
    __syncthreads();
    const u32 npair = nst >> 1;
    for (u32 k = 0; k < npair; k++) {
        const u32 l = DIT ? 2 * k : nst - 2 - 2 * k;
        const u32 s = lo + l;
        const Fr* t_lo = tws + (((size_t)1 << s) - 1);
        const Fr* t_hi = tws + (((size_t)2 << s) - 1);
        for (u32 q = threadIdx.x; q < (tile_elems >> 2); q += nthr) {
            u32 c = q & (cols - 1), rr = q >> cols_bits;
            u32 r0 = ((rr >> l) << (l + 2)) | (rr & ((1u << l) - 1u));
            u32 j = (u32)((base | ((size_t)r0 << lo) | c) & (((size_t)1 << s) - 1));
            Fr wc = fr_load(&t_lo[j]);
            Fr wa = fr_load(&t_hi[j]);
            Fr wb = fr_load(&t_hi[j + (1u << s)]);
            u32 i0 = (r0 << cols_bits) | c, st = 1u << (l + cols_bits);
            Fr x0 = lds[i0], x1 = lds[i0 + st], x2 = lds[i0 + 2 * st], x3 = lds[i0 + 3 * st];
            if (DIT) {
                Fr v = Fr::mul(x1, wc), u = Fr::mul(x3, wc);
                x1 = Fr::sub(x0, v); x0 = Fr::add(x0, v);
                x3 = Fr::sub(x2, u); x2 = Fr::add(x2, u);
                v = Fr::mul(x2, wa); u = Fr::mul(x3, wb);
                x2 = Fr::sub(x0, v); x0 = Fr::add(x0, v);
                x3 = Fr::sub(x1, u); x1 = Fr::add(x1, u);
            } else {
                Fr v = Fr::sub(x0, x2), u = Fr::sub(x1, x3);
                x0 = Fr::add(x0, x2); x1 = Fr::add(x1, x3);
                x2 = Fr::mul(v, wa); x3 = Fr::mul(u, wb);
                v = Fr::sub(x0, x1); u = Fr::sub(x2, x3);
                x0 = Fr::add(x0, x1); x2 = Fr::add(x2, x3);
                x1 = Fr::mul(v, wc); x3 = Fr::mul(u, wc);
            }
            lds[i0] = x0; lds[i0 + st] = x1; lds[i0 + 2 * st] = x2; lds[i0 + 3 * st] = x3;
        }
        __syncthreads();
    }
    if (nst & 1) {
        const u32 l = DIT ? nst - 1 : 0;
        const u32 s = lo + l;
        const Fr* t_lo = tws + (((size_t)1 << s) - 1);
        for (u32 q = threadIdx.x; q < (tile_elems >> 1); q += nthr) {
            u32 c = q & (cols - 1), rr = q >> cols_bits;
            u32 r0 = ((rr >> l) << (l + 1)) | (rr & ((1u << l) - 1u));
            u32 j = (u32)((base | ((size_t)r0 << lo) | c) & (((size_t)1 << s) - 1));
            Fr w = fr_load(&t_lo[j]);
            u32 i0 = (r0 << cols_bits) | c, st = 1u << (l + cols_bits);
            Fr x0 = lds[i0], x1 = lds[i0 + st];
            if (DIT) {
                Fr v = Fr::mul(x1, w);
                lds[i0] = Fr::add(x0, v);
                lds[i0 + st] = Fr::sub(x0, v);
            } else {
                lds[i0] = Fr::add(x0, x1);
                lds[i0 + st] = Fr::mul(Fr::sub(x0, x1), w);
            }
        }
        __syncthreads();
    }
    for (u32 e = threadIdx.x; e < tile_elems; e += nthr) {
        u32 r = e >> cols_bits, c = e & (cols - 1);
        size_t gi = base | ((size_t)r << lo) | c;
        Fr x = lds[e];
        if (post & 2) x = Fr::mul(x, pow_from_tables(pw, logn ? (__brev((u32)gi) >> (32 - logn)) : 0u, logn));
        if (post & 4) x = Fr::sub(x, Fr::mul(fr_load(&sub[gi]), kc));
        if (post & 1) x = Fr::mul(x, scale);
        fr_store(&vec[gi], x);
    }
}

template <class Fr>
__global__ void k_scale_pow(Fr* __restrict__ data, size_t stride_vec, const Fr* __restrict__ pw, Fr scale,
                            u32 logn, int bitrev_index, int use_pow) {
    size_t pos = (size_t)blockIdx.x * blockDim.x + threadIdx.x;
    if (pos >> logn) return;
    Fr* vec = data + (size_t)blockIdx.y * stride_vec;
    Fr x = fr_load(&vec[pos]);
    x = Fr::mul(x, scale);
    if (use_pow) {
        u32 j = bitrev_index ? (logn ? (__brev((u32)pos) >> (32 - logn)) : 0u) : (u32)pos;
        x = Fr::mul(x, pow_from_tables(pw, j, logn));
    }
    fr_store(&vec[pos], x);
}

template <class Fr>
__global__ void k_bitrev(Fr* __restrict__ data, u32 logn) {
    size_t pos = (size_t)blockIdx.x * blockDim.x + threadIdx.x;
    if (pos >> logn) return;
    u32 r = logn ? (__brev((u32)pos) >> (32 - logn)) : 0u;
    if (r > pos) {
        Fr a = fr_load(&data[pos]), b = fr_load(&data[r]);
        fr_store(&data[pos], b);
        fr_store(&data[r], a);
    }
}

template <class Fr>
__global__ void k_mul_pointwise(Fr* __restrict__ a, const Fr* __restrict__ b, size_t m) {
    size_t i = (size_t)blockIdx.x * blockDim.x + threadIdx.x;
    if (i >= m) return;
    fr_store(&a[i], Fr::mul(fr_load(&a[i]), fr_load(&b[i])));
}

#endif

}
```

### hekaton_system_amd/csrc/ntt_host.cuh

```cuda
#pragma once
#include "curve_ops_impl.cuh"
#include "ntt.cuh"
#include "ntt_plan.h"
#include "csr.cuh"

namespace hk {

template <class Fr>
static Fr host_halve(const Fr& a) {
    u32 t[Fr::N + 1];
    u64 c = 0;
    bool odd = a.v[0] & 1;
    for (int i = 0; i < Fr::N; i++) {
        c += (u64)a.v[i] + (odd ? Fr::Params::MOD[i] : 0u);
        t[i] = (u32)c;
        c >>= 32;
    }
    t[Fr::N] = (u32)c;
    Fr r;
    for (int i = 0; i < Fr::N; i++) r.v[i] = (t[i] >> 1) | (t[i + 1] << 31);
    return r;
}
template <class Fr>
static Fr host_from_limbs(const u32* l) {
    Fr r;
    for (int i = 0; i < Fr::N; i++) r.v[i] = l[i];
    return r;
}

struct NttTables {
    std::mutex mu;
    u32 log_table = 0;
    void* tw_fwd = nullptr;
    void* tw_inv = nullptr;
    void* pw_g = nullptr;
    void* pw_ginv = nullptr;
    std::vector<void*> retired;
};

template <class C>
struct NttHost {
    typedef typename C::Fr Fr;

    static hk_status ensure(hk_ctx* ctx, u32 log_m, NttTables** out) {
        if (log_m > C::TWO_ADICITY) return HK_ERR_DOMAIN_TOO_LARGE;
        std::unique_lock<std::mutex> lk(ctx->mu);
        if (!ctx->ntt) ctx->ntt = new NttTables();
        NttTables* T = ctx->ntt;
        lk.unlock();
        std::unique_lock<std::mutex> tl(T->mu);
        *out = T;
        if (T->log_table >= log_m && T->tw_fwd) return HK_OK;
        u32 L = log_m < 16 ? 16 : log_m;
        if (L > C::TWO_ADICITY) L = C::TWO_ADICITY;
        HK_HIP(hipSetDevice(ctx->device));
        std::vector<Fr> sq(32), sqi(32);
        Fr w = host_from_limbs<Fr>(C::ROOT);
        for (u32 k = 0; k < C::TWO_ADICITY - L; k++) w = Fr::sqr(w);
        Fr winv = Fr::one();
        for (u32 k = 0; k < L; k++) {
            sq[k] = w;
            winv = Fr::mul(winv, w);
            w = Fr::sqr(w);
        }
        Fr t = winv;
        for (u32 k = 0; k < L; k++) { sqi[k] = t; t = Fr::sqr(t); }
        const u32 NG = 3 * POW_TABLE_BITS;
        std::vector<Fr> gs(NG), gis(NG);
        Fr g = host_from_limbs<Fr>(C::GEN), gi = host_from_limbs<Fr>(C::GEN_INV);
        for (u32 k = 0; k < NG; k++) { gs[k] = g; gis[k] = gi; g = Fr::sqr(g); gi = Fr::sqr(gi); }
        Fr *d_sq = nullptr, *tmp = nullptr, *tf = nullptr, *ti = nullptr, *pg = nullptr, *pgi = nullptr;
        size_t half = (size_t)1 << (L - 1), full = (size_t)1 << L;
        HK_HIP(hipMalloc((void**)&d_sq, sizeof(Fr) * (64 + 2 * NG)));
        HK_HIP(hipMalloc((void**)&tmp, sizeof(Fr) * half));
        HK_HIP(hipMalloc((void**)&tf, sizeof(Fr) * full));
        HK_HIP(hipMalloc((void**)&ti, sizeof(Fr) * full));
        HK_HIP(hipMalloc((void**)&pg, sizeof(Fr) * 3 * POW_TABLE_SIZE));
        HK_HIP(hipMalloc((void**)&pgi, sizeof(Fr) * 3 * POW_TABLE_SIZE));
        HK_HIP(hipMemcpy(d_sq, sq.data(), sizeof(Fr) * 32, hipMemcpyHostToDevice));
        HK_HIP(hipMemcpy(d_sq + 32, sqi.data(), sizeof(Fr) * 32, hipMemcpyHostToDevice));
        HK_HIP(hipMemcpy(d_sq + 64, gs.data(), sizeof(Fr) * NG, hipMemcpyHostToDevice));
        HK_HIP(hipMemcpy(d_sq + 64 + NG, gis.data(), sizeof(Fr) * NG, hipMemcpyHostToDevice));
        u32 blocks = (u32)((half + 255) / 256), blocks_full = (u32)((full + 255) / 256);
        hipLaunchKernelGGL((k_pow_table<Fr>), dim3(blocks), dim3(256), 0, 0, tmp, d_sq, (u32)half, L - 1);
        hipLaunchKernelGGL((k_stage_tables<Fr>), dim3(blocks_full), dim3(256), 0, 0, tf, tmp, L);
        hipLaunchKernelGGL((k_pow_table<Fr>), dim3(blocks), dim3(256), 0, 0, tmp, d_sq + 32, (u32)half, L - 1);
        hipLaunchKernelGGL((k_stage_tables<Fr>), dim3(blocks_full), dim3(256), 0, 0, ti, tmp, L);
        for (u32 lvl = 0; lvl < 3; lvl++) {
            hipLaunchKernelGGL((k_pow_table<Fr>), dim3(POW_TABLE_SIZE / 256), dim3(256), 0, 0, pg + POW_TABLE_SIZE * lvl,
                               d_sq + 64 + POW_TABLE_BITS * lvl, (u32)POW_TABLE_SIZE, (u32)POW_TABLE_BITS);
            hipLaunchKernelGGL((k_pow_table<Fr>), dim3(POW_TABLE_SIZE / 256), dim3(256), 0, 0, pgi + POW_TABLE_SIZE * lvl,
                               d_sq + 64 + NG + POW_TABLE_BITS * lvl, (u32)POW_TABLE_SIZE, (u32)POW_TABLE_BITS);
        }
        HK_HIP(hipGetLastError());
        HK_HIP(hipDeviceSynchronize());
        HK_HIP(hipFree(d_sq));
        HK_HIP(hipFree(tmp));
        for (void* p : {T->tw_fwd, T->tw_inv, T->pw_g, T->pw_ginv})
            if (p) T->retired.push_back(p);
        T->tw_fwd = tf; T->tw_inv = ti; T->pw_g = pg; T->pw_ginv = pgi;
        T->log_table = L;
        return HK_OK;
    }

    static Fr size_inv(u32 log_m) {
        Fr x = Fr::one();
        for (u32 k = 0; k < log_m; k++) x = host_halve(x);
        return x;
    }
    static Fr vanishing_inv_on_coset(u32 log_m) {
        Fr g = host_from_limbs<Fr>(C::GEN);
        for (u32 k = 0; k < log_m; k++) g = Fr::sqr(g);
        return fp_inv(Fr::sub(g, Fr::one()));
    }

    struct Post {
        int post = 0;
        u32 nvec = 0xffffffffu;
        const Fr* scale = nullptr;
        const Fr* pw = nullptr;
        const Fr* sub = nullptr;
        const Fr* kc = nullptr;
    };

    static hk_status passes(hipStream_t s, Fr* data, size_t stride, u32 batch, u32 logn, const Fr* tws, int dit,
                            const Post& ep = Post()) {
        if (logn == 0) return HK_OK;
        static const u32 tile_log = [] {
            const char* e = getenv("HK_NTT_TILE_LOG");
            return ntt_plan_tile_log(e ? (u32)atoi(e) : NTT_PLAN_TILE_LOG);
        }();
        static const u32 upper_max = [] {
            const char* e = getenv("HK_NTT_UPPER_MAX");
            return ntt_plan_upper_max(e ? (u32)atoi(e) : NTT_PLAN_UPPER_MAX, tile_log);
        }();
        const u32 threads = 1u << (tile_log - 2);
        NttPass ps[NTT_PLAN_MAX_PASSES];
        int np = ntt_pass_plan(logn, tile_log, upper_max, ps);
        Fr one = Fr::one();
        for (int k = 0; k < np; k++) {
            const NttPass& p = dit ? ps[k] : ps[np - 1 - k];
            u32 tile_log = p.nst + p.cols_bits;
            dim3 grid(1u << (logn - tile_log), batch);
            size_t lds = sizeof(Fr) << tile_log;
            bool last = k == np - 1;
            int pp = last ? ep.post : 0;
            const Fr& sc = (pp & 1) ? *ep.scale : one;
            const Fr& kc = (pp & 4) ? *ep.kc : one;
            if (dit)
                hipLaunchKernelGGL((k_ntt_pass4<Fr, 1>), grid, dim3(threads), lds, s, data, stride, tws, logn, p.lo,
                                   p.nst, p.cols_bits, pp, ep.nvec, sc, ep.pw, ep.sub, kc);
            else
                hipLaunchKernelGGL((k_ntt_pass4<Fr, 0>), grid, dim3(threads), lds, s, data, stride, tws, logn, p.lo,
                                   p.nst, p.cols_bits, pp, ep.nvec, sc, ep.pw, ep.sub, kc);
        }
        HK_HIP(hipGetLastError());
        return HK_OK;
    }

    static hk_status scale(hipStream_t s, Fr* data, size_t stride, u32 batch, u32 logn, const Fr* pw,
                           const Fr& sc, int bitrev_index, int use_pow) {
        size_t n = (size_t)1 << logn;
        hipLaunchKernelGGL((k_scale_pow<Fr>), dim3((u32)((n + 255) / 256), batch), dim3(256), 0, s, data,
                           stride, pw, sc, logn, bitrev_index, use_pow);
        HK_HIP(hipGetLastError());
        return HK_OK;
    }
    static hk_status bitrev(hipStream_t s, Fr* data, u32 logn) {
        size_t n = (size_t)1 << logn;
        hipLaunchKernelGGL((k_bitrev<Fr>), dim3((u32)((n + 255) / 256)), dim3(256), 0, s, data, logn);
        HK_HIP(hipGetLastError());
        return HK_OK;
    }
};

template <class C>
hk_status Ops<C>::ntt(hk_ctx* ctx, void* data, unsigned log_m, int inverse, int coset) {
    typedef NttHost<C> N;
    NttTables* T;
    HK_TRY(N::ensure(ctx, log_m, &T));
    LaneGuard g(ctx);
    Lane* L = g.lane;
    if (!L) return HK_ERR_DEVICE;
    size_t n = (size_t)1 << log_m;
    Fr* stage;
    HK_TRY(L->carve([&](Carve& c) { stage = c.n<Fr>(n); }));
    bool dev = is_device_ptr(data);
    Fr* d = (Fr*)data;
    if (!dev) {
        d = stage;
        HK_HIP(hipMemcpyAsync(d, data, n * sizeof(Fr), hipMemcpyHostToDevice, L->stream));
    }
    hipStream_t s = L->stream;
    if (!inverse) {
        if (coset) HK_TRY(N::scale(s, d, n, 1, log_m, (const Fr*)T->pw_g, Fr::one(), 0, 1));
        HK_TRY(N::passes(s, d, n, 1, log_m, (const Fr*)T->tw_fwd, 0));
        HK_TRY(N::bitrev(s, d, log_m));
    } else {
        Fr minv = N::size_inv(log_m);
        typename N::Post ep;
        ep.post = coset ? 3 : 1;
        ep.scale = &minv;
        ep.pw = (const Fr*)T->pw_ginv;
        HK_TRY(N::passes(s, d, n, 1, log_m, (const Fr*)T->tw_inv, 0, ep));
        HK_TRY(N::bitrev(s, d, log_m));
    }
    if (!dev) HK_HIP(hipMemcpyAsync(data, d, n * sizeof(Fr), hipMemcpyDeviceToHost, s));
    return L->settle();
}

template <class C>
struct QapHost {
    typedef typename C::Fr Fr;
    typedef NttHost<C> N;

    static u32 domain_log(size_t n_c, size_t n_inst) {
        size_t need = n_c + n_inst;
        u32 lg = 0;
        while (((size_t)1 << lg) < need) lg++;
        return lg;
    }
    static hk_status run(hipStream_t s, NttTables* T, const CsrDev& A, const CsrDev& B, const CsrDev& Cm,
                         size_t n_inst, size_t n_c, const Fr* z, Fr* abc, u32 log_m) {
        size_t m = (size_t)1 << log_m;
        const CsrDev* Ms[3] = {&A, &B, &Cm};
        for (int k = 0; k < 3; k++) {
            hipLaunchKernelGGL((k_spmv<Fr>), dim3((u32)((m + 255) / 256)), dim3(256), 0, s,
                               Ms[k]->row_ptr, Ms[k]->col, (const Fr*)Ms[k]->val, z, abc + k * m,
                               (u32)n_c, k == 0 ? (u32)n_inst : 0u, (u32)m);
        }
        const Fr* tinv = (const Fr*)T->tw_inv;
        const Fr* tfwd = (const Fr*)T->tw_fwd;
        typename N::Post e1;
        e1.post = 2;
        e1.nvec = 2;
        e1.pw = (const Fr*)T->pw_g;
        HK_TRY(N::passes(s, abc, m, 3, log_m, tinv, 0, e1));
        HK_TRY(N::passes(s, abc, m, 2, log_m, tfwd, 1));
        hipLaunchKernelGGL((k_mul_pointwise<Fr>), dim3((u32)((m + 255) / 256)), dim3(256), 0, s, abc, abc + m, m);
        Fr minv = N::size_inv(log_m);
        Fr mm = fp_inv(Fr::mul(minv, minv));
        Fr k = Fr::mul(N::vanishing_inv_on_coset(log_m), Fr::mul(minv, Fr::mul(minv, minv)));
        typename N::Post e2;
        e2.post = 2 | 4 | 1;
        e2.pw = (const Fr*)T->pw_ginv;
        e2.sub = abc + 2 * m;
        e2.kc = &mm;
        e2.scale = &k;
        HK_TRY(N::passes(s, abc, m, 1, log_m, tinv, 0, e2));
        HK_HIP(hipGetLastError());
        return HK_OK;
    }
    static hk_status run_eval(hipStream_t s, NttTables* T, const CsrDev& A, const CsrDev& B, size_t n_inst, size_t n_c,
                              const Fr* z, Fr* ab, u32 log_m) {
        size_t m = (size_t)1 << log_m;
        const CsrDev* Ms[2] = {&A, &B};
        for (int k = 0; k < 2; k++)
            hipLaunchKernelGGL((k_spmv<Fr>), dim3((u32)((m + 255) / 256)), dim3(256), 0, s,
                               Ms[k]->row_ptr, Ms[k]->col, (const Fr*)Ms[k]->val, z, ab + k * m,
                               (u32)n_c, k == 0 ? (u32)n_inst : 0u, (u32)m);
        typename N::Post e1;
        e1.post = 2;
        e1.nvec = 2;
        e1.pw = (const Fr*)T->pw_g;
        HK_TRY(N::passes(s, ab, m, 2, log_m, (const Fr*)T->tw_inv, 0, e1));
        HK_TRY(N::passes(s, ab, m, 2, log_m, (const Fr*)T->tw_fwd, 1));
        hipLaunchKernelGGL((k_mul_pointwise<Fr>), dim3((u32)((m + 255) / 256)), dim3(256), 0, s, ab, ab + m, m);
        HK_HIP(hipGetLastError());
        return HK_OK;
    }
};

template <class C>
hk_status Ops<C>::witness_map(hk_ctx* ctx, const hk_csr* A, const hk_csr* B, const hk_csr* Cm, size_t n_inst,
                              size_t n_c, const void* z, size_t n_v, void* h_out, size_t h_cap,
                              size_t* m_out) {
    typedef QapHost<C> Q;
    if (A->n_rows != n_c || B->n_rows != n_c || Cm->n_rows != n_c || n_inst > n_v || n_inst < 1) return HK_ERR_ARG;
    if (!csr_host_ok(A) || !csr_host_ok(B) || !csr_host_ok(Cm)) return HK_ERR_ARG;
    u32 log_m = Q::domain_log(n_c, n_inst);
    if (log_m > C::TWO_ADICITY) return HK_ERR_DOMAIN_TOO_LARGE;
    size_t m = (size_t)1 << log_m;
    if (m_out) *m_out = m;
    if (h_cap < m) return HK_ERR_LEN;
    NttTables* T;
    HK_TRY(NttHost<C>::ensure(ctx, log_m, &T));
    R1csStage stage(A, B, Cm, n_v, sizeof(Fr));
    Staged zin = staged(z, n_v * sizeof(Fr));
    LaneGuard g(ctx);
    Lane* L = g.lane;
    if (!L) return HK_ERR_DEVICE;
    Fr* abc;
    HK_TRY(L->carve([&](Carve& c) {
        stage.carve(c);
        stage_carve(c, &zin, 1);
        abc = c.n<Fr>(3 * m);
    }));
    CsrDev D[3];
    HK_TRY(stage.upload(L, D));
    HK_TRY(stage_upload(L, &zin, 1));
    HK_TRY(Q::run(L->stream, T, D[0], D[1], D[2], n_inst, n_c, (const Fr*)zin.p, abc, log_m));
    HK_TRY(NttHost<C>::bitrev(L->stream, abc, log_m));
    HK_HIP(hipMemcpyAsync(h_out, abc, m * sizeof(Fr),
                          is_device_ptr(h_out) ? hipMemcpyDeviceToDevice : hipMemcpyDeviceToHost, L->stream));
    return L->settle();
}

template <class C>
void Ops<C>::ctx_release(hk_ctx* ctx) {
    for (auto& e : ctx->fb_cache)
        if (e.table) (void)hipFree(e.table);
    ctx->fb_cache.clear();
    if (!ctx->ntt) return;
    NttTables* T = ctx->ntt;
    for (void* p : {T->tw_fwd, T->tw_inv, T->pw_g, T->pw_ginv})
        if (p) (void)hipFree(p);
    for (void* p : T->retired) (void)hipFree(p);
    delete T;
    ctx->ntt = nullptr;
}

}
```

### hekaton_system_amd/csrc/pk.cuh

```cuda
#pragma once
#include "ntt_host.cuh"
#include "csr.cuh"
#include "h_basis.cuh"

namespace hk {

template <class C>
struct PkImpl {
    typedef typename C::Fr Fr;
    typedef typename C::Fq Fq;
    typedef typename C::Fq2 Fq2;
    u32 n_v = 0, n_inst = 0, n_c = 0, n_stages = 0, n_ext = 0, n_extra = 0;
    MsmPlan plan_z;
    Affine<Fq>* a_tab = nullptr;
    Affine<Fq>* b1_tab = nullptr;
    Affine<Fq2>* b2_tab = nullptr;
    bool a_compact = false, b_compact = false;
    u32 a_n = 0, b_n = 0;
    u32 *a_rank = nullptr, *b_rank = nullptr;
    MsmPlan plan_a, plan_b;
    Affine<Fq>* l_tab = nullptr;
    u32 l_n = 0, l_off = 0;
    bool has_qap = false;
    bool h_eval = false;
// ... 116 lines not shown
        auto cleanup = [&]() { for (void* q : tmp) (void)hipFree(q); tmp.clear(); };
        auto tfail = [&](hk_status e) { cleanup(); return fail(e); };
        auto talloc = [&](void** q, size_t b) { if (hipMalloc(q, b ? b : 16) != hipSuccess) { (void)hipGetLastError(); return false; } tmp.push_back(*q); return true; };
        if (!talloc((void**)&sa, g1 * (nq + 1)) || !talloc((void**)&sb1, g1 * (nq + 1)) || !talloc((void**)&sb2, g2 * (nq + 1)) ||
            !talloc((void**)&flags, 4 * (nq + 1)))
            return tfail(HK_ERR_NOMEM);
        if (nq) {
            if (hipMemcpy(sa, a_g + g1, g1 * nq, h2d_kind(a_g)) != hipSuccess) return tfail(HK_ERR_DEVICE);
            if (hipMemcpy(sb1, b_g + g1, g1 * nq, h2d_kind(b_g)) != hipSuccess) return tfail(HK_ERR_DEVICE);
            if (hipMemcpy(sb2, b_h + g2, g2 * nq, h2d_kind(b_h)) != hipSuccess) return tfail(HK_ERR_DEVICE);
        }
        static const char* dens_env = getenv("HK_B_COMPACT_BELOW");
        double thr = dens_env ? atof(dens_env) / 100.0 : 0.75;
        auto select = [&](const Affine<Fq>* staged, bool* compact, u32* n_out, MsmPlan* plan, u32** idx_d, u32** rank_d) -> hk_status {
            std::vector<u32> idx;
            if (nq) {
                hipLaunchKernelGGL((k_mark_noninf<Fq>), dim3((u32)((nq + 255) / 256)), dim3(256), 0, s0, staged, flags, (u32)nq);
                std::vector<u32> hf(nq);
                if (hipMemcpy(hf.data(), flags, 4 * nq, hipMemcpyDeviceToHost) != hipSuccess) return HK_ERR_DEVICE;
                for (size_t i = 0; i < nq; i++) if (hf[i]) idx.push_back((u32)i);
            }
            *compact = msm_compact_rule(nq, idx.size(), thr);
            *idx_d = *rank_d = nullptr;
            if (!*compact) {
                *n_out = pk->n_ext;
                *plan = pz;
                return HK_OK;
            }
            for (u32 e = 0; e < pk->n_extra; e++) idx.push_back((u32)nq + e);
            *n_out = (u32)idx.size();
            *plan = msm_sub_plan(pz, *n_out, ctx->max_lanes0);
            std::vector<u32> rank(pk->n_ext);
            msm_rank_table(idx.data(), idx.size(), rank.data(), rank.size());
            if (!talloc((void**)idx_d, 4 * idx.size())) return HK_ERR_NOMEM;
            void* dr = nullptr;
            if (hipMalloc(&dr, 4 * rank.size()) != hipSuccess) { (void)hipGetLastError(); return HK_ERR_NOMEM; }
            pk->owned.push_back(dr);
            pk->bytes += 4 * rank.size();
            *rank_d = (u32*)dr;
            if (hipMemcpy(*idx_d, idx.data(), 4 * idx.size(), hipMemcpyHostToDevice) != hipSuccess) return HK_ERR_DEVICE;
            if (hipMemcpy(dr, rank.data(), 4 * rank.size(), hipMemcpyHostToDevice) != hipSuccess) return HK_ERR_DEVICE;
            return HK_OK;
        };
        u32 *a_idx = nullptr, *b_idx = nullptr;
        if ((st = select(sa, &pk->a_compact, &pk->a_n, &pk->plan_a, &a_idx, &pk->a_rank)) != HK_OK) return tfail(st);
        if ((st = select(sb1, &pk->b_compact, &pk->b_n, &pk->plan_b, &b_idx, &pk->b_rank)) != HK_OK) return tfail(st);
        if ((st = pk_alloc_table(pk->owned, pk->bytes, pz.F, pk->a_n, &pk->a_tab)) != HK_OK) return tfail(st);
        if ((st = pk_alloc_table(pk->owned, pk->bytes, pz.F, pk->b_n, &pk->b1_tab)) != HK_OK) return tfail(st);
        if ((st = pk_alloc_table(pk->owned, pk->bytes, pz.F, pk->b_n, &pk->b2_tab)) != HK_OK) return tfail(st);
        if (hipMemset(pk->a_tab, 0, g1 * pk->a_n) != hipSuccess || hipMemset(pk->b1_tab, 0, g1 * pk->b_n) != hipSuccess ||
            hipMemset(pk->b2_tab, 0, g2 * pk->b_n) != hipSuccess)
            return tfail(HK_ERR_DEVICE);
        if (pk->a_compact) {
            hipLaunchKernelGGL((k_gather<Affine<Fq>>), dim3((pk->a_n + 255) / 256), dim3(256), 0, s0, pk->a_tab, (const Affine<Fq>*)sa, (const u32*)a_idx, pk->a_n, (u32)nq);
        } else if (nq) {
            if (hipMemcpy(pk->a_tab, sa, g1 * nq, hipMemcpyDeviceToDevice) != hipSuccess) return tfail(HK_ERR_DEVICE);
        }
        if (pk->b_compact) {
            u32 blocks = (pk->b_n + 255) / 256;
            hipLaunchKernelGGL((k_gather<Affine<Fq>>), dim3(blocks), dim3(256), 0, s0, pk->b1_tab, (const Affine<Fq>*)sb1, (const u32*)b_idx, pk->b_n, (u32)nq);
            hipLaunchKernelGGL((k_gather<Affine<Fq2>>), dim3(blocks), dim3(256), 0, s0, pk->b2_tab, (const Affine<Fq2>*)sb2, (const u32*)b_idx, pk->b_n, (u32)nq);
        } else if (nq) {
            if (hipMemcpy(pk->b1_tab, sb1, g1 * nq, hipMemcpyDeviceToDevice) != hipSuccess) return tfail(HK_ERR_DEVICE);
            if (hipMemcpy(pk->b2_tab, sb2, g2 * nq, hipMemcpyDeviceToDevice) != hipSuccess) return tfail(HK_ERR_DEVICE);
        }
        u32 r_slot = pk->a_n - pk->n_extra + 0, s_slot = pk->b_n - pk->n_extra + 1;
        if (hipMemcpy(pk->a_tab + r_slot, delta_last_g, g1, h2d_kind(deltas)) != hipSuccess) return tfail(HK_ERR_DEVICE);
        if (hipMemcpy(pk->b1_tab + s_slot, delta_last_g, g1, h2d_kind(deltas)) != hipSuccess) return tfail(HK_ERR_DEVICE);
        if (hipMemcpy(pk->b2_tab + s_slot, d->last_delta_h, g2, h2d_kind(d->last_delta_h)) != hipSuccess) return tfail(HK_ERR_DEVICE);
        if (hipDeviceSynchronize() != hipSuccess) return tfail(HK_ERR_DEVICE);
        cleanup();
        PK_TRY(MsmRun<Fq>::build_tables(s0, pk->a_tab, pk->a_n, pz.F, shift));
        PK_TRY(MsmRun<Fq>::build_tables(s0, pk->b1_tab, pk->b_n, pz.F, shift));
        PK_TRY(MsmRun<Fq2>::build_tables(s0, pk->b2_tab, pk->b_n, pz.F, shift));
    }
    size_t n1 = d->ck_len[k];
    const size_t l_rows = pk->h_eval ? n_v - 1 : n1;
    pk->l_n = (u32)l_rows + pk->n_extra;
    pk->l_off = (u32)(n_v - 1 - l_rows);
    if ((st = pk_alloc_table(pk->owned, pk->bytes, pz.F, pk->l_n, &pk->l_tab)) != HK_OK) return fail(st);
    PK_HIP(hipMemset(pk->l_tab, 0, g1 * pk->l_n));
    if (n1 && !pk->h_eval) PK_HIP(hipMemcpy(pk->l_tab, d->ck_stage[k], g1 * n1, h2d_kind(d->ck_stage[k])));
    {
        std::vector<Affine<Fq>> dh(k + 1);
        PK_HIP(hipMemcpy(dh.data(), deltas, g1 * (k + 1), is_device_ptr(deltas) ? hipMemcpyDeviceToHost : hipMemcpyHostToHost));
        std::vector<Affine<Fq>> neg(1 + k);
        neg[0] = dh[k].is_inf() ? dh[k] : ec_neg(dh[k]);
        for (u32 i = 0; i < k; i++) neg[1 + i] = dh[i].is_inf() ? dh[i] : ec_neg(dh[i]);
        PK_HIP(hipMemcpy(pk->l_tab + l_rows + 2, neg.data(), g1 * (1 + k), hipMemcpyHostToDevice));
    }
    if (!pk->h_eval) PK_TRY(MsmRun<Fq>::build_tables(s0, pk->l_tab, pk->l_n, pz.F, shift));
    for (u32 sidx = 0; sidx < pk->n_stages; sidx++) {
        size_t n = d->ck_len[sidx] + 1;
        MsmPlan p = make_plan(n);
        Affine<Fq>* tab;
        if ((st = pk_alloc_table(pk->owned, pk->bytes, p.F, n, &tab)) != HK_OK) return fail(st);
        if (n > 1) PK_HIP(hipMemcpy(tab, d->ck_stage[sidx], g1 * (n - 1), h2d_kind(d->ck_stage[sidx])));
        PK_HIP(hipMemcpy(tab + n - 1, delta_last_g, g1, h2d_kind(deltas)));
        PK_TRY(MsmRun<Fq>::build_tables(s0, tab, (u32)n, p.F, p.c * p.WP));
        pk->plan_ck.push_back(p);
        pk->ck_tab.push_back(tab);
        pk->ck_n.push_back((u32)n);
    }
    {
        void* p1; void* p2;
        PK_HIP(hipMalloc(&p1, g1 * 5)); pk->owned.push_back(p1);
        PK_HIP(hipMalloc(&p2, g2 * 2)); pk->owned.push_back(p2);
        pk->consts_g1 = (Affine<Fq>*)p1; pk->consts_g2 = (Affine<Fq2>*)p2;
        PK_HIP(hipMemset(pk->consts_g1 + 4, 0, g1));
        PK_HIP(hipMemcpy(pk->consts_g1 + 0, a_g, g1, h2d_kind(a_g)));
        PK_HIP(hipMemcpy(pk->consts_g1 + 1, d->alpha_g, g1, h2d_kind(d->alpha_g)));
        PK_HIP(hipMemcpy(pk->consts_g1 + 2, b_g, g1, h2d_kind(b_g)));
        PK_HIP(hipMemcpy(pk->consts_g1 + 3, d->beta_g, g1, h2d_kind(d->beta_g)));
        PK_HIP(hipMemcpy(pk->consts_g2 + 0, b_h, g2, h2d_kind(b_h)));
        PK_HIP(hipMemcpy(pk->consts_g2 + 1, d->beta_h, g2, h2d_kind(d->beta_h)));
    }
    if (has_qap) {
        if (d->A->n_rows != d->n_constraints || d->B->n_rows != d->n_constraints ||
            d->C->n_rows != d->n_constraints)
            return fail(HK_ERR_LEN);
        pk->log_m = QapHost<C>::domain_log(d->n_constraints, d->n_inst);
        if (pk->log_m > C::TWO_ADICITY || pk->log_m > (u32)MSM_ENTRY_GROUP_SHIFT) return fail(HK_ERR_DOMAIN_TOO_LARGE);
        size_t m = (size_t)1 << pk->log_m;
        if (d->h_len + 1 != m) return fail(HK_ERR_LEN);
        const hk_csr* Ms[3] = {d->A, d->B, d->C};
        if (!csr_host_ok(d->A) || !csr_host_ok(d->B) || !csr_host_ok(d->C)) return fail(HK_ERR_ARG);
        for (int i = 0; i < 3; i++) {
            void *rp, *cl, *vl;
            PK_HIP(hipMalloc(&rp, 8 * (Ms[i]->n_rows + 1))); pk->owned.push_back(rp);
            PK_HIP(hipMalloc(&cl, 4 * Ms[i]->nnz + 16)); pk->owned.push_back(cl);
            PK_HIP(hipMalloc(&vl, sizeof(Fr) * Ms[i]->nnz + 16)); pk->owned.push_back(vl);
            PK_HIP(hipMemcpy(rp, Ms[i]->row_ptr, 8 * (Ms[i]->n_rows + 1), h2d_kind(Ms[i]->row_ptr)));
            if (Ms[i]->nnz) {
                PK_HIP(hipMemcpy(cl, Ms[i]->col, 4 * Ms[i]->nnz, h2d_kind(Ms[i]->col)));
                PK_HIP(hipMemcpy(vl, Ms[i]->val_mont, sizeof(Fr) * Ms[i]->nnz, h2d_kind(Ms[i]->val_mont)));
            }
            pk->csr[i] = {(const u64*)rp, (const u32*)cl, vl, Ms[i]->n_rows, Ms[i]->nnz};
            pk->bytes += 8 * (Ms[i]->n_rows + 1) + (4 + sizeof(Fr)) * Ms[i]->nnz;
        }
        {
            void* flag = nullptr;
            PK_HIP(hipMalloc(&flag, 256)); pk->owned.push_back(flag);
            PK_TRY(r1cs_validate(s0, pk->csr, n_v, (u32*)flag));
        }
        pk->plan_h = make_plan(m);
        if ((st = pk_alloc_table(pk->owned, pk->bytes, pk->plan_h.F, m, &pk->h_tab)) != HK_OK) return fail(st);
        const Affine<Fq>* src = (const Affine<Fq>*)d->h_g;
        if (!is_device_ptr(d->h_g)) {
            PK_HIP(hipMalloc(&staging, g1 * (d->h_len ? d->h_len : 1)));
            PK_HIP(hipMemcpy(staging, d->h_g, g1 * d->h_len, hipMemcpyHostToDevice));
            src = (const Affine<Fq>*)staging;
        }
        NttTables* T;
        PK_TRY(NttHost<C>::ensure(ctx, pk->log_m, &T));
        if (pk->h_eval) {
            PK_HIP(hipMalloc(&hb_tmp, g1 * (m + n_v)));
            Affine<Fq>*gd = (Affine<Fq>*)hb_tmp, *cd = gd + m;
            PK_TRY(HBasis<C>::transform(ctx, T, src, (u32)d->h_len, pk->log_m, pk->h_tab, gd));
            PK_TRY(HBasis<C>::c_columns(ctx, pk->csr[2], n_v, pk->log_m, gd, d->ck_stage[k], n1, cd));
            if (nq) PK_HIP(hipMemcpy(pk->l_tab, cd + 1, g1 * nq, hipMemcpyDeviceToDevice));
            PK_HIP(hipMemcpy(pk->consts_g1 + 4, cd, g1, hipMemcpyDeviceToDevice));
            (void)hipFree(hb_tmp); hb_tmp = nullptr;
            PK_TRY(MsmRun<Fq>::build_tables(s0, pk->l_tab, pk->l_n, pz.F, shift));
        } else {
            hipLaunchKernelGGL((k_pk_bitrev_copy<Fq>), dim3((u32)((m + 255) / 256)), dim3(256), 0, s0, pk->h_tab,
                               src, (u32)d->h_len, pk->log_m);
            PK_HIP(hipDeviceSynchronize());
        }
        if (staging) { (void)hipFree(staging); staging = nullptr; }
        PK_TRY(MsmRun<Fq>::build_tables(s0, pk->h_tab, (u32)m, pk->plan_h.F, pk->plan_h.c * pk->plan_h.WP));
        pk->has_qap = true;
    }
    PK_HIP(hipDeviceSynchronize());
    *out = h;
    return HK_OK;
}

#undef PK_HIP
#undef PK_TRY

template <class C>
void Ops<C>::pk_free(hk_pk* h) {
    if (!h) return;
    PkImpl<C>* pk = (PkImpl<C>*)h->impl;
    (void)hipSetDevice(h->ctx->device);
    (void)hipDeviceSynchronize();
    for (void* p : pk->owned) (void)hipFree(p);
    delete pk;
    delete h;
}

}
```

### hekaton_system_amd/csrc/prove_impl.cuh

```cuda
#pragma once
#include "ntt_host.cuh"
#include "pk.cuh"

namespace hk {

template <class Fr>
__global__ void k_prep_ext(Fr* __restrict__ ext, u32 ext_stride, const Fr* __restrict__ rs_kappas, u32 rs_stride,
                           u32 n_kappas, u32 batch, u32* __restrict__ c0, u32* __restrict__ c1, u32 nb0, u32 nb1) {
    u32 gt = blockIdx.x * blockDim.x + threadIdx.x, stride = gridDim.x * blockDim.x;
    for (u32 i = gt; i < nb0; i += stride) c0[i] = 0;
    for (u32 i = gt; i < nb1; i += stride) c1[i] = 0;
    if (gt >= batch) return;
    Fr* e = ext + (size_t)gt * ext_stride;
    const Fr* rk = rs_kappas + (size_t)gt * rs_stride;
    Fr r = fr_load(&rk[0]), s = fr_load(&rk[1]);
    fr_store(&e[0], r);
    fr_store(&e[1], s);
    fr_store(&e[2], Fr::mul(r, s));
    for (u32 i = 0; i < n_kappas; i++) fr_store(&e[3 + i], fr_load(&rk[2 + i]));
}

template <class Fr, class Fq, class Fq2>
__global__ void k_finish_ab(const XYZZ<Fq>* __restrict__ res_g1_all, const XYZZ<Fq2>* __restrict__ res_g2_all,
                            const Affine<Fq>* __restrict__ c1, const Affine<Fq2>* __restrict__ c2, const Fr* __restrict__ rs_all,
// ... 41 lines not shown
                Jac<Fq> e = Jac<Fq>::from_affine(q);
                tab[t][0] = e;
                HK_NOUNROLL for (int i = 2; i <= SPLIT_TABLE; i++) {
                    Jac<Fq> prev = (i & 1) ? tab[t][i - 2] : tab[t][i / 2 - 1];
                    e = (i & 1) ? jac_madd_ni(prev, q) : jac_dbl_ni(prev);
                    tab[t][i - 1] = e;
                }
                HK_NOUNROLL for (int d = ND - 1; d >= 0; d--) {
                    int dig = split_digit(m, d);
                    if (dig == 0 && acc.is_inf()) continue;
                    HK_NOUNROLL for (int r4 = 0; r4 < 4; r4++) acc = jac_dbl_ni(acc);
                    if (dig != 0) {
                        Jac<Fq> e2 = tab[t][(dig < 0 ? -dig : dig) - 1];
                        if (dig < 0) e2.y = Fq::neg(e2.y);
                        acc = jac_add_ni(acc, e2);
                    }
                }
            }
            part[t] = acc;
        }
        __syncthreads();
        if (t == 0) {
            Jac<Fq> sum = part[0];
            HK_NOUNROLL for (int i = 1; i < 4; i++) sum = jac_add_ni(sum, part[i]);
            XYZZ<Fq> Cc = XYZZ<Fq>::inf();
            if (!sum.is_inf()) {
                Cc.x = sum.x; Cc.y = sum.y;
                Cc.zz = Fq::sqr(sum.z);
                Cc.zzz = Fq::mul(Cc.zz, sum.z);
            }
            st_vec(part_c, ec_madd_ni(ec_add_ni(Cc, ld_vec(&res_g1[2])), ld_vec(&c1[4])));
        }
    }
}

static_assert(HK_PROVE_BATCH_CHUNK <= 64, "k_finish_c covers a chunk with one wave");
template <class Fq>
__global__ void __launch_bounds__(64) k_finish_c(const XYZZ<Fq>* __restrict__ part_c, const XYZZ<Fq>* __restrict__ res_g1_all,
                                                 Affine<Fq>* __restrict__ out_c, u32 batch) {
    const u32 pr = threadIdx.x;
    if (pr >= batch) return;
    XYZZ<Fq> Cc = ec_add_ni(ld_vec(&part_c[pr]), ld_vec(&res_g1_all[4 * (size_t)pr + 3]));
    st_vec(&out_c[pr], ec_to_affine(Cc));
}

template <class C>
size_t Ops<C>::finish_private_bytes() {
    size_t ab = hk_private_bytes_of((const void*)k_finish_ab<Fr, Fq, Fq2>);
    size_t c = hk_private_bytes_of((const void*)k_finish_c<Fq>);
    size_t hb = HBasis<C>::private_bytes();
    return std::max(std::max(ab, c), hb);
}

template <class C>
hk_status Ops<C>::commit(hk_ctx* ctx, const hk_pk* h, size_t stage, const void* w, size_t n,
                         const void* kappa, void* out) {
    if (h->ctx != ctx) return HK_ERR_ARG;
    PkImpl<C>* pk = (PkImpl<C>*)h->impl;
    if (stage >= pk->n_stages) return HK_ERR_ARG;
    if (n + 1 != pk->ck_n[stage]) return HK_ERR_LEN;
    if (n && !w) return HK_ERR_ARG;
    if ((n + 1) * EndoOf<Fq>::K <= SPLIT_MAX_LANES && !is_device_ptr(out) && !getenv("HK_MSM_NO_SMALL"))
        return commit_batch(ctx, h, stage, w, n, kappa, 1, out);
    LaneGuard g(ctx);
    Lane* L = g.lane;
    if (!L) return HK_ERR_DEVICE;
    OneMsm<Fq> msm{false, &pk->plan_ck[stage], (u32)(n + 1)};
    Fr* sc;
    HK_TRY(L->carve([&](Carve& c) { sc = c.n<Fr>(n + 1); msm.carve(c); }));
    hipStream_t s = L->stream;
    bool prof = ctx->profiling;
    if (prof) HK_HIP(hipEventRecord(L->ev[0], s));
    if (n) HK_HIP(hipMemcpyAsync(sc, w, n * sizeof(Fr), h2d_kind(w), s));
    HK_HIP(hipMemcpyAsync(sc + n, kappa, sizeof(Fr), hipMemcpyHostToDevice, s));
    HK_TRY(msm.run(s, pk->ck_tab[stage], sc, 1, out, hipMemcpyDeviceToHost, prof ? L->ev[20] : nullptr, prof ? L->ev[21] : nullptr));
    if (prof) HK_HIP(hipEventRecord(L->ev[1], s));
    HK_TRY(L->settle());
    if (prof) {
        memset(&L->timings, 0, sizeof(L->timings));
        L->timings.total_ms = ev_ms(L->ev[0], L->ev[1]);
        L->timings.accum_kernel_ms = ev_ms(L->ev[20], L->ev[21]);
        L->timings.accum_kernel_launches = 1;
    }
    return HK_OK;
}

template <class C>
hk_status Ops<C>::commit_batch(hk_ctx* ctx, const hk_pk* h, size_t stage, const void* w, size_t n, const void* kappas,
                               size_t batch, void* out) {
    if (h->ctx != ctx) return HK_ERR_ARG;
    PkImpl<C>* pk = (PkImpl<C>*)h->impl;
    if (stage >= pk->n_stages) return HK_ERR_ARG;
    if (n + 1 != pk->ck_n[stage]) return HK_ERR_LEN;
    if (batch == 0) return HK_OK;
    if ((n && !w) || !kappas || !out) return HK_ERR_ARG;
    const size_t seg = n + 1, tot = seg * batch;
    if (tot * EndoOf<Fq>::K > SPLIT_MAX_LANES || is_device_ptr(kappas) || getenv("HK_MSM_NO_SMALL")) {
        if (is_device_ptr(kappas) || is_device_ptr(out)) return HK_ERR_ARG;
        for (size_t b = 0; b < batch; b++)
            HK_TRY(commit(ctx, h, stage, n ? (const char*)w + b * n * sizeof(Fr) : nullptr, n, (const char*)kappas + b * sizeof(Fr),
                          (char*)out + b * sizeof(Affine<Fq>)));
        return HK_OK;
    }
    LaneGuard g(ctx);
    Lane* L = g.lane;
    if (!L) return HK_ERR_DEVICE;
    Fr* sc;
    XYZZ<Fq>*xy, *tab, *res;
    Fq* pref;
    Affine<Fq>* aff;
    HK_TRY(L->carve([&](Carve& c) {
        sc = c.n<Fr>(tot);
        xy = c.n<XYZZ<Fq>>(tot);
        tab = (XYZZ<Fq>*)c.take(endo_tab_bytes<Fq>(tot));
        res = c.n<XYZZ<Fq>>(batch);
        pref = c.n<Fq>(batch);
        aff = c.n<Affine<Fq>>(batch);
    }));
    hipStream_t s = L->stream;
    bool prof = ctx->profiling;
    if (prof) HK_HIP(hipEventRecord(L->ev[0], s));
    if (n) HK_HIP(hipMemcpy2DAsync(sc, seg * sizeof(Fr), w, n * sizeof(Fr), n * sizeof(Fr), batch, h2d_kind(w), s));
    HK_HIP(hipMemcpy2DAsync(sc + n, seg * sizeof(Fr), kappas, sizeof(Fr), sizeof(Fr), batch, hipMemcpyHostToDevice, s));
    HK_TRY(MsmRun<Fq>::small_msm_rows(s, pk->ck_tab[stage], sc, (u32)seg, (u32)batch, tab, xy, res));
    HK_TRY(MsmRun<Fq>::batch_affine(s, res, aff, pref, (u32)batch));
    HK_HIP(hipMemcpyAsync(out, aff, batch * sizeof(Affine<Fq>), is_device_ptr(out) ? hipMemcpyDeviceToDevice : hipMemcpyDeviceToHost, s));
    if (prof) HK_HIP(hipEventRecord(L->ev[1], s));
    HK_TRY(L->settle());
    if (prof) {
        memset(&L->timings, 0, sizeof(L->timings));
        L->timings.total_ms = ev_ms(L->ev[0], L->ev[1]);
    }
    return HK_OK;
}

template <class C>
hk_status Ops<C>::prove_batch(hk_ctx* ctx, const hk_pk* h, size_t n_v, size_t n_kappas, const ProveRow* rows, size_t batch) {
    typedef QapHost<C> Q;
    if (h->ctx != ctx) return HK_ERR_ARG;
    PkImpl<C>* pk = (PkImpl<C>*)h->impl;
    if (!pk->has_qap) return HK_ERR_ARG;
    if (n_v != pk->n_v) return HK_ERR_LEN;
    if (n_kappas + 1 != pk->n_stages) return HK_ERR_LEN;
    if (batch == 0) return HK_OK;
    if (!rows) return HK_ERR_ARG;
    for (size_t b = 0; b < batch; b++) {
        const ProveRow& w = rows[b];
        if (!w.z || !w.r || !w.s || !w.a || !w.b || !w.c || (n_kappas && !w.kappas)) return HK_ERR_ARG;
    }
    LaneGuard g(ctx, ProveLaneTag{});
    Lane* L = g.lane;
    if (!L) return HK_ERR_DEVICE;
    NttTables* T;
    HK_TRY(NttHost<C>::ensure(ctx, pk->log_m, &T));
    const MsmPlan &pz = pk->plan_z, &ph = pk->plan_h, &pa = pk->plan_a, &pb = pk->plan_b;
    const size_t m = (size_t)1 << pk->log_m, fr = sizeof(Fr), rs_stride = 2 + n_kappas;
    const size_t h_stride = (pk->h_eval ? 2 : 3) * m;
    std::vector<char> z_dev(batch);
    bool any_host = false;
    for (size_t b = 0; b < batch; b++) {
        z_dev[b] = is_device_ptr(rows[b].z);
        any_host = any_host || !z_dev[b];
    }
    Fr *zext, *small, *zt, *abc;
    SortBufs sb, sbh, sba, sbb;
    typename MsmRun<Fq>::Bufs rbA, rbB1, rbL, rbh;
    typename MsmRun<Fq2>::Bufs rb2;
    XYZZ<Fq>* res1;
    XYZZ<Fq2>* res2;
    Affine<Fq> *oa, *oc;
    Affine<Fq2>* ob;
    XYZZ<Fq>* pc;
    auto chunk_bufs = [&](Carve& c, u32 nb) {
        zext = c.n<Fr>((size_t)pk->n_ext * nb);
        small = c.n<Fr>(rs_stride * nb);
        zt = any_host ? c.n<Fr>(n_v * nb) : nullptr;
        MsmSort<Fr>::alloc(c, pz, &sb, nb);
        MsmSort<Fr>::alloc(c, ph, &sbh, nb);
        if (pk->a_compact) MsmSort<Fr>::alloc_sub(c, pz, pa, &sba, nb);
        if (pk->b_compact) MsmSort<Fr>::alloc_sub(c, pz, pb, &sbb, nb);
        MsmRun<Fq>::alloc(c, pa, &rbA, nb);
        MsmRun<Fq>::alloc(c, pb, &rbB1, nb);
        MsmRun<Fq>::alloc(c, pz, &rbL, nb);
        MsmRun<Fq>::alloc(c, ph, &rbh, nb);
        MsmRun<Fq2>::alloc(c, pb, &rb2, nb);
        res1 = c.n<XYZZ<Fq>>(4 * (size_t)nb);
        res2 = c.n<XYZZ<Fq2>>(nb);
        oa = c.n<Affine<Fq>>(nb);
        oc = c.n<Affine<Fq>>(nb);
        ob = c.n<Affine<Fq2>>(nb);
        pc = c.n<XYZZ<Fq>>(nb);
        abc = c.n<Fr>(h_stride * nb);
    };
    size_t chunk = batch < (size_t)HK_PROVE_BATCH_CHUNK ? batch : (size_t)HK_PROVE_BATCH_CHUNK;
    if (chunk > 1) {
        size_t free_b = 0, total_b = 0;
        if (hipMemGetInfo(&free_b, &total_b) != hipSuccess) { (void)hipGetLastError(); free_b = 0; }
        size_t avail = free_b + L->arena_cap;
        auto chunk_bytes = [&](size_t nb) { Carve c; chunk_bufs(c, (u32)nb); return c.off; };
        while (chunk > 1 && chunk_bytes(chunk) > avail) chunk--;
    }
    std::vector<unsigned char> rsk(batch * rs_stride * fr);
    for (size_t b = 0; b < batch; b++) {
        unsigned char* row = rsk.data() + b * rs_stride * fr;
        memcpy(row, rows[b].r, fr);
        memcpy(row + fr, rows[b].s, fr);
        if (n_kappas) memcpy(row + 2 * fr, rows[b].kappas, n_kappas * fr);
    }
    std::vector<Affine<Fq>> ha(chunk), hc(chunk);
    std::vector<Affine<Fq2>> hb(chunk);
    std::vector<const Fr*> zd(chunk);
    const bool prof = ctx->profiling;
    hipEvent_t* ev = L->ev;
    hk_timings acc;
    memset(&acc, 0, sizeof(acc));
    static const EndoSplit<2> endo_g1 = EndoOf<Fq>::split();
    hipStream_t rs[PROVE_ROLES];
    for (int r = 0; r < PROVE_ROLES; r++) rs[r] = L->stream_at(prove_role_stream(L->n_streams, (ProveRole)r));
    hipStream_t s = rs[ROLE_MAIN];
    auto wait = [](hipStream_t to, hipEvent_t e, hipStream_t from) -> hk_status {
        if (to != from) HK_HIP(hipStreamWaitEvent(to, e, 0));
        return HK_OK;
    };
    for (size_t b0 = 0; b0 < batch; b0 += chunk) {
        const u32 nb = (u32)std::min(chunk, batch - b0);
        HK_TRY(L->carve([&](Carve& c) { chunk_bufs(c, nb); }));
        hipEvent_t ev_start = b0 ? ev[9] : ev[0];
        if (prof) HK_HIP(hipEventRecord(ev_start, s));
        for (u32 j = 0; j < nb; j++) {
            if (z_dev[b0 + j]) zd[j] = (const Fr*)rows[b0 + j].z;
            else {
                HK_HIP(hipMemcpyAsync(zt + (size_t)j * n_v, rows[b0 + j].z, n_v * fr, hipMemcpyHostToDevice, s));
                zd[j] = zt + (size_t)j * n_v;
            }
            if (n_v > 1)
                HK_HIP(hipMemcpyAsync(zext + (size_t)j * pk->n_ext, zd[j] + 1, (n_v - 1) * fr, hipMemcpyDeviceToDevice, s));
        }
        HK_HIP(hipMemcpyAsync(small, rsk.data() + b0 * rs_stride * fr, nb * rs_stride * fr, hipMemcpyHostToDevice, s));
        hipLaunchKernelGGL((k_prep_ext<Fr>), dim3(64), dim3(256), 0, s, zext + (n_v - 1), pk->n_ext, (const Fr*)small,
                           (u32)rs_stride, (u32)n_kappas, nb, sb.count, sbh.count, pz.NB * nb, ph.NB * nb);
        hipStream_t sB1 = rs[ROLE_B1], sB2 = rs[ROLE_B2], sL = rs[ROLE_L], sH = rs[ROLE_H];
        hipEvent_t ev_z = ev[16], ev_sorted = ev[17];
        HK_HIP(hipEventRecord(ev_z, s));
        auto submit_h = [&]() -> hk_status {
            HK_TRY(wait(sH, ev_z, s));
            if (prof) HK_HIP(hipEventRecord(ev[5], sH));
            for (u32 j = 0; j < nb; j++) {
                if (pk->h_eval)
                    HK_TRY(Q::run_eval(sH, T, pk->csr[0], pk->csr[1], pk->n_inst, pk->n_c, zd[j], abc + j * h_stride, pk->log_m));
                else
                    HK_TRY(Q::run(sH, T, pk->csr[0], pk->csr[1], pk->csr[2], pk->n_inst, pk->n_c, zd[j],
                                  abc + j * h_stride, pk->log_m));
            }
            if (prof) HK_HIP(hipEventRecord(ev[6], sH));
            HK_TRY(MsmSort<Fr>::run(sH, ph, (const u32*)abc, 1, sbh, true, nb, h_stride));
            HK_TRY(MsmRun<Fq>::run(sH, ph, pk->h_tab, (u32)m, 0, sbh, rbh, res1 + 3, prof ? ev[12] : nullptr,
                                   prof ? ev[13] : nullptr, nb, 4));
            HK_HIP(hipEventRecord(ev[7], sH));
            return HK_OK;
        };
        const bool h_first = L->n_streams >= 3;
        if (h_first) HK_TRY(submit_h());
        HK_TRY(MsmSort<Fr>::run(s, pz, (const u32*)zext, 1, sb, true, nb, pk->n_ext));
        HK_HIP(hipEventRecord(ev_sorted, s));
        if (prof) HK_HIP(hipEventRecord(ev[1], s));
        HK_TRY(wait(sL, ev_sorted, s));
        const SortBufs *sbA = &sb, *sbB = &sb;
        HK_TRY(wait(sB1, ev_sorted, s));
        if (pk->b_compact) {
            HK_TRY(MsmSort<Fr>::sublist(sB1, pz, sb, pb, pk->b_rank, sbb, nb));
            HK_HIP(hipEventRecord(ev[28], sB1));
            HK_TRY(wait(sB2, ev[28], sB1));
            sbB = &sbb;
        } else {
            HK_TRY(wait(sB2, ev_sorted, s));
        }
        HK_TRY(MsmRun<Fq2>::run(sB2, pb, pk->b2_tab, pk->b_n, 0, *sbB, rb2, res2, nullptr, nullptr, nb, 1));
        HK_HIP(hipEventRecord(ev[4], sB2));
        HK_TRY(MsmRun<Fq>::run(sB1, pb, pk->b1_tab, pk->b_n, 0, *sbB, rbB1, res1 + 1, prof ? ev[22] : nullptr,
                               prof ? ev[23] : nullptr, nb, 4));
        HK_HIP(hipEventRecord(ev[3], sB1));
        HK_TRY(MsmRun<Fq>::run(sL, pz, pk->l_tab, pk->l_n, pk->l_off, sb, rbL, res1 + 2, prof ? ev[24] : nullptr,
                               prof ? ev[25] : nullptr, nb, 4));
        HK_HIP(hipEventRecord(ev[18], sL));
        if (pk->a_compact) {
            HK_TRY(MsmSort<Fr>::sublist(s, pz, sb, pa, pk->a_rank, sba, nb));
            sbA = &sba;
        }
        HK_TRY(MsmRun<Fq>::run(s, pa, pk->a_tab, pk->a_n, 0, *sbA, rbA, res1 + 0, prof ? ev[26] : nullptr,
                               prof ? ev[27] : nullptr, nb, 4));
        if (prof) HK_HIP(hipEventRecord(ev[2], s));
        HK_TRY(wait(s, ev[3], sB1));
        HK_TRY(wait(s, ev[4], sB2));
        HK_TRY(wait(s, ev[18], sL));
        hipLaunchKernelGGL((k_finish_ab<Fr, Fq, Fq2>), dim3(3, nb), dim3(64), 0, s, res1, res2, pk->consts_g1, pk->consts_g2,
                           (const Fr*)small, (u32)rs_stride, oa, ob, pc, endo_g1);
        HK_HIP(hipGetLastError());
        if (!h_first) HK_TRY(submit_h());
        HK_TRY(wait(s, ev[7], sH));
        if (prof) HK_HIP(hipEventRecord(ev[19], s));
        hipLaunchKernelGGL((k_finish_c<Fq>), dim3(1), dim3(64), 0, s, (const XYZZ<Fq>*)pc, (const XYZZ<Fq>*)res1, oc, nb);
        HK_HIP(hipGetLastError());
        HK_HIP(hipMemcpyAsync(ha.data(), oa, nb * sizeof(Affine<Fq>), hipMemcpyDeviceToHost, s));
        HK_HIP(hipMemcpyAsync(hb.data(), ob, nb * sizeof(Affine<Fq2>), hipMemcpyDeviceToHost, s));
        HK_HIP(hipMemcpyAsync(hc.data(), oc, nb * sizeof(Affine<Fq>), hipMemcpyDeviceToHost, s));
        if (prof) HK_HIP(hipEventRecord(ev[8], s));
        HK_TRY(L->settle());
        for (u32 j = 0; j < nb; j++) {
            memcpy(rows[b0 + j].a, &ha[j], sizeof(Affine<Fq>));
            memcpy(rows[b0 + j].b, &hb[j], sizeof(Affine<Fq2>));
            memcpy(rows[b0 + j].c, &hc[j], sizeof(Affine<Fq>));
        }
        if (prof) {
            acc.digits_ms += ev_ms(ev_start, ev[1]);
            acc.msm_a_ms += ev_ms(ev[1], ev[2]);
            acc.msm_b_g1_ms += ev_ms(ev[1], ev[3]);
            acc.msm_b_g2_ms += ev_ms(ev[1], ev[4]);
            acc.msm_l_ms += ev_ms(ev[1], ev[18]);
            acc.witness_map_ms += ev_ms(ev[5], ev[6]);
            acc.msm_h_ms += ev_ms(ev[6], ev[7]);
            acc.finish_ms += ev_ms(ev[19], ev[8]);
            float kh = ev_ms(ev[12], ev[13]);
            acc.accum_h_ms += kh;
            acc.accum_kernel_ms += kh + ev_ms(ev[22], ev[23]) + ev_ms(ev[24], ev[25]) + ev_ms(ev[26], ev[27]);
            acc.accum_kernel_launches += 4;
        }
    }
    if (prof) {
        acc.total_ms = ev_ms(ev[0], ev[8]);
        acc.batch_proofs = (uint32_t)chunk;
        L->timings = acc;
    }
    return HK_OK;
}

}
```

Baseline: 135.4.

## Fuse H-poly coset NTT seam and move pointwise product into MSM histogram

In the h_eval path, the inverse NTT, coset scaling and forward NTT are restructured. The lowest-level passes of both transforms are merged into a single LDS-resident seam kernel that uses precomputed coset-twisted twiddle tables, which skips the separate pw_g scaling post-pass. The A·B pointwise multiply is removed and folded into the MSM histogram kernel, which multiplies the two scalar vectors on load; the Montgomery factor is compensated by adjusting c0 in the h-basis. The aim is fewer full-memory passes over the 2m vectors, at the cost of a new coset table per log_m and a new testing API.

```diff
diff --git a/hekaton_system_amd/csrc/curve_ops_impl.cuh b/hekaton_system_amd/csrc/curve_ops_impl.cuh
--- a/hekaton_system_amd/csrc/curve_ops_impl.cuh
+++ b/hekaton_system_amd/csrc/curve_ops_impl.cuh
@@ -167,6 +167,7 @@
     hk_status trace_sort(hk_ctx*, uint32_t, const void*, size_t, void*, uint32_t*) override;
     hk_status stage0_witness(hk_ctx*, const uint32_t*, uint32_t, uint32_t, const void*, const void*, const uint32_t*, size_t,
                              void*) override;
+    hk_status pk_witness_map_eval(hk_ctx*, const hk_pk*, const void*, size_t, void*, size_t) override;
     hk_status r1cs_check(hk_ctx*, const hk_csr*, const hk_csr*, const hk_csr*, const void*, size_t, size_t, hk_r1cs_verdict*,
                          uint32_t*, void*, size_t) override;
     hk_status pk_r1cs_check(hk_ctx*, const hk_pk*, const void*, size_t, size_t, hk_r1cs_verdict*, uint32_t*, void*, size_t) override;
diff --git a/hekaton_system_amd/csrc/h_basis.cuh b/hekaton_system_amd/csrc/h_basis.cuh
--- a/hekaton_system_amd/csrc/h_basis.cuh
+++ b/hekaton_system_amd/csrc/h_basis.cuh
@@ -109,7 +109,9 @@
         hipStream_t s = L->stream;
         static const EndoSplit<2> E = EndoOf<Fq>::split();
         Fr minv = N::size_inv(log_m), zinv = N::vanishing_inv_on_coset(log_m);
-        Fr c1 = Fr::mul(zinv, minv), c0 = Fr::mul(c1, Fr::mul(minv, minv));
+        Fr rinv = Fr::zero();
+        rinv.v[0] = 1;
+        Fr c1 = Fr::mul(zinv, minv), c0 = Fr::mul(Fr::mul(c1, Fr::mul(minv, minv)), rinv);
         hipLaunchKernelGGL((k_hb_load<Fr, Fq>), dim3((u32)((m + 63) / 64), 2), dim3(64), 0, s, h_g, h_len, log_m,
                            (const Fr*)T->pw_ginv, c0, c1, E, x);
         for (u32 st = 0; st < log_m; st++)
diff --git a/hekaton_system_amd/csrc/hk_core.hip b/hekaton_system_amd/csrc/hk_core.hip
--- a/hekaton_system_amd/csrc/hk_core.hip
+++ b/hekaton_system_amd/csrc/hk_core.hip
@@ -634,6 +634,10 @@
     if (!ctx || !pk) return HK_ERR_ARG;
     return ctx->ops->pk_r1cs_check(ctx, pk, z_mont, n_v, batch, verdicts, bad_rows, bad_vals, cap);
 }
+hk_status hk_pk_witness_map_eval(hk_ctx* ctx, const hk_pk* pk, const void* z_mont, size_t n_v, void* out, size_t cap) {
+    if (!ctx || !pk) return HK_ERR_ARG;
+    return ctx->ops->pk_witness_map_eval(ctx, pk, z_mont, n_v, out, cap);
+}
 hk_status hk_sha_tree(hk_ctx* ctx, const void* leaves, uint32_t n_sub, uint32_t ns, uint32_t n_portals, const hk_sha_tree_out* out) {
     if (!ctx || !leaves || !out) return HK_ERR_ARG;
     return ctx->ops->sha_tree(ctx, leaves, n_sub, ns, n_portals, out);
diff --git a/hekaton_system_amd/csrc/hk_internal.h b/hekaton_system_amd/csrc/hk_internal.h
--- a/hekaton_system_amd/csrc/hk_internal.h
+++ b/hekaton_system_amd/csrc/hk_internal.h
@@ -9,6 +9,7 @@
 #include <vector>
 
 #include "../../include/hekaton.h"
+#include "../../include/hekaton_testing.h"
 #include "coalesce.h"
 #include "msm.cuh"
 #include "stream_plan.h"
@@ -198,6 +199,7 @@
                                  uint32_t* perm_out) = 0;
     virtual hk_status stage0_witness(hk_ctx*, const uint32_t* offsets, uint32_t n_sub, uint32_t n_portals, const void* time_entries,
                                      const void* addr_entries, const uint32_t* sub_index, size_t batch, void* w_out) = 0;
+    virtual hk_status pk_witness_map_eval(hk_ctx*, const hk_pk*, const void* z, size_t n_v, void* out, size_t cap) = 0;
     virtual hk_status r1cs_check(hk_ctx*, const hk_csr* A, const hk_csr* B, const hk_csr* C, const void* z, size_t n_v, size_t batch,
                                  hk_r1cs_verdict* verdicts, uint32_t* bad_rows, void* bad_vals, size_t cap) = 0;
     virtual hk_status pk_r1cs_check(hk_ctx*, const hk_pk*, const void* z, size_t n_v, size_t batch, hk_r1cs_verdict* verdicts,
diff --git a/hekaton_system_amd/csrc/msm.cuh b/hekaton_system_amd/csrc/msm.cuh
--- a/hekaton_system_amd/csrc/msm.cuh
+++ b/hekaton_system_amd/csrc/msm.cuh
@@ -59,8 +59,7 @@
 #if defined(__HIPCC__)
 
 template <class Fr>
-__device__ __forceinline__ void msm_load_scalar(const u32* scalars, size_t i, int is_mont,
-                                                const MsmPlan& p, u32 (&sp)[10]) {
+__device__ __forceinline__ Fr msm_load_fr(const u32* scalars, size_t i) {
     Fr s;
     const uint4* src = reinterpret_cast<const uint4*>(scalars + i * Fr::N);
 #pragma unroll
@@ -68,7 +67,14 @@
         uint4 v = src[k];
         s.v[4 * k] = v.x; s.v[4 * k + 1] = v.y; s.v[4 * k + 2] = v.z; s.v[4 * k + 3] = v.w;
     }
-    if (is_mont) s = Fr::from_mont(s);
+    return s;
+}
+template <class Fr>
+__device__ __forceinline__ void msm_load_scalar(const u32* scalars, size_t i, int is_mont,
+                                                const MsmPlan& p, u32 (&sp)[10], const u32* scalars2 = nullptr) {
+    Fr s = msm_load_fr<Fr>(scalars, i);
+    if (scalars2) s = Fr::canon(Fr::mul(s, msm_load_fr<Fr>(scalars2, i)));
+    else if (is_mont) s = Fr::from_mont(s);
     u64 carry = 0;
 #pragma unroll
     for (int k = 0; k < Fr::N; k++) {
@@ -107,14 +113,14 @@
 }
 
 template <class Fr>
-__global__ void __launch_bounds__(MSM_SORT_THREADS)
-k_msm_hist(const u32* __restrict__ scalars_all, size_t scalar_stride_words, int is_mont, MsmPlan p,
-           u32* __restrict__ count_all, short* __restrict__ digits_all) {
+__device__ __forceinline__ void msm_hist_block(const u32* __restrict__ scalars_all, const u32* __restrict__ scalars2_all,
+                                               size_t scalar_stride_words, int is_mont, const MsmPlan& p,
+                                               u32* __restrict__ count_all, short* __restrict__ digits_all, u32* h) {
     const size_t pr = blockIdx.y;
     const u32* __restrict__ scalars = scalars_all + pr * scalar_stride_words;
+    const u32* __restrict__ scalars2 = scalars2_all ? scalars2_all + pr * scalar_stride_words : nullptr;
     u32* __restrict__ count = count_all + pr * p.NB;
     short* __restrict__ digits = digits_all + pr * msm_digits_stride(p);
-    __shared__ u32 h[MSM_LDS_COUNTERS];
     for (u32 b = threadIdx.x; b < p.NB; b += blockDim.x) h[b] = 0;
     __syncthreads();
     size_t base = (size_t)blockIdx.x * p.chunk;
@@ -122,7 +128,7 @@
         size_t i = base + k;
         if (i >= p.n) break;
         u32 sp[10];
-        msm_load_scalar<Fr>(scalars, i, is_mont, p, sp);
+        msm_load_scalar<Fr>(scalars, i, is_mont, p, sp, scalars2);
         switch (p.c) {
 #define HK_HIST_C(C) case C: msm_hist_scalar<Fr, C>(sp, i, p, digits, h); break;
             HK_HIST_C(3) HK_HIST_C(4) HK_HIST_C(5) HK_HIST_C(6) HK_HIST_C(7) HK_HIST_C(8) HK_HIST_C(9) HK_HIST_C(10)
@@ -135,6 +141,20 @@
         u32 v = h[b];
         if (v) atomicAdd(&count[b], v);
     }
+}
+template <class Fr>
+__global__ void __launch_bounds__(MSM_SORT_THREADS)
+k_msm_hist(const u32* __restrict__ scalars_all, size_t scalar_stride_words, int is_mont, MsmPlan p,
+           u32* __restrict__ count_all, short* __restrict__ digits_all) {
+    __shared__ u32 h[MSM_LDS_COUNTERS];
+    msm_hist_block<Fr>(scalars_all, nullptr, scalar_stride_words, is_mont, p, count_all, digits_all, h);
+}
+template <class Fr>
+__global__ void __launch_bounds__(MSM_SORT_THREADS)
+k_msm_hist_mul(const u32* __restrict__ x_all, const u32* __restrict__ y_all, size_t scalar_stride_words, MsmPlan p,
+               u32* __restrict__ count_all, short* __restrict__ digits_all) {
+    __shared__ u32 h[MSM_LDS_COUNTERS];
+    msm_hist_block<Fr>(x_all, y_all, scalar_stride_words, 0, p, count_all, digits_all, h);
 }
 
 template <int UNUSED>
diff --git a/hekaton_system_amd/csrc/msm_driver.cuh b/hekaton_system_amd/csrc/msm_driver.cuh
--- a/hekaton_system_amd/csrc/msm_driver.cuh
+++ b/hekaton_system_amd/csrc/msm_driver.cuh
@@ -29,7 +29,8 @@
     static hk_status sublist(hipStream_t s, const MsmPlan& src, const SortBufs& sb_src, const MsmPlan& dst, const u32* rank,
                              const SortBufs& sb_dst, u32 batch = 1);
     static hk_status run(hipStream_t s, const MsmPlan& p, const u32* scalars_d, int is_mont,
-                         const SortBufs& sb, bool count_is_zero = false, u32 batch = 1, size_t scalar_stride = 0);
+                         const SortBufs& sb, bool count_is_zero = false, u32 batch = 1, size_t scalar_stride = 0,
+                         const u32* scalars2_d = nullptr);
 };
 
 template <class F>
diff --git a/hekaton_system_amd/csrc/msm_driver_impl.cuh b/hekaton_system_amd/csrc/msm_driver_impl.cuh
--- a/hekaton_system_amd/csrc/msm_driver_impl.cuh
+++ b/hekaton_system_amd/csrc/msm_driver_impl.cuh
@@ -64,15 +64,19 @@
 
 template <class Fr>
 hk_status MsmSort<Fr>::run(hipStream_t s, const MsmPlan& p, const u32* scalars_d, int is_mont,
-                           const SortBufs& sb, bool count_is_zero, u32 batch, size_t scalar_stride) {
+                           const SortBufs& sb, bool count_is_zero, u32 batch, size_t scalar_stride, const u32* scalars2_d) {
     if (p.NB > (u32)MSM_LDS_COUNTERS || p.c < 3 || p.c > 16) return HK_ERR_ARG;
     if (batch == 0 || batch > 65535u) return HK_ERR_ARG;
     if (!count_is_zero) HK_HIP(hipMemsetAsync(sb.count, 0, sizeof(u32) * p.NB * batch, s));
     u32 blocks = (p.n + p.chunk - 1) / p.chunk;
     if (blocks == 0) blocks = 1;
     const size_t words = scalar_stride * (sizeof(Fr) / sizeof(u32));
-    hipLaunchKernelGGL((k_msm_hist<Fr>), dim3(blocks, batch), dim3(MSM_SORT_THREADS), 0, s,
-                       scalars_d, words, is_mont, p, sb.count, sb.digits);
+    if (scalars2_d)
+        hipLaunchKernelGGL((k_msm_hist_mul<Fr>), dim3(blocks, batch), dim3(MSM_SORT_THREADS), 0, s,
+                           scalars_d, scalars2_d, words, p, sb.count, sb.digits);
+    else
+        hipLaunchKernelGGL((k_msm_hist<Fr>), dim3(blocks, batch), dim3(MSM_SORT_THREADS), 0, s,
+                           scalars_d, words, is_mont, p, sb.count, sb.digits);
     HK_DBG(s, "k_msm_hist");
     hipLaunchKernelGGL((k_msm_scan<0>), dim3(batch), dim3(1024), 0, s, sb.count, sb.start, sb.cursor, p.NB);
     HK_DBG(s, "k_msm_scan");
diff --git a/hekaton_system_amd/csrc/ntt.cuh b/hekaton_system_amd/csrc/ntt.cuh
--- a/hekaton_system_amd/csrc/ntt.cuh
+++ b/hekaton_system_amd/csrc/ntt.cuh
@@ -52,6 +52,14 @@
     u32 s = 31 - __clz((u32)(i + 1));
     size_t j = i + 1 - ((size_t)1 << s);
     fr_store(&tws[i], fr_load(&tw[j << (log_table - s - 1)]));
+}
+
+template <class Fr>
+__global__ void k_coset_tables(Fr* __restrict__ out, const Fr* __restrict__ tws, const Fr* __restrict__ gsq, u32 logn) {
+    size_t i = (size_t)blockIdx.x * blockDim.x + threadIdx.x;
+    if ((i + 1) >> logn) return;
+    u32 s = 31 - __clz((u32)(i + 1));
+    fr_store(&out[i], Fr::mul(fr_load(&tws[i]), fr_load(&gsq[logn - 1 - s])));
 }
 
 template <class Fr, int DIT>
@@ -141,6 +149,101 @@
     }
 }
 
+template <class Fr, int DIT>
+__device__ __forceinline__ void seam_step4(Fr* lds, const Fr* __restrict__ tws, u32 l, u32 tile_elems) {
+    const Fr* t_lo = tws + ((1u << l) - 1u);
+    const Fr* t_hi = tws + ((2u << l) - 1u);
+    for (u32 q = threadIdx.x; q < (tile_elems >> 2); q += blockDim.x) {
+        u32 j = q & ((1u << l) - 1u);
+        u32 i0 = ((q >> l) << (l + 2)) | j, st = 1u << l;
+        Fr wc = fr_load(&t_lo[j]);
+        Fr wa = fr_load(&t_hi[j]);
+        Fr wb = fr_load(&t_hi[j + st]);
+        Fr x0 = lds[i0], x1 = lds[i0 + st], x2 = lds[i0 + 2 * st], x3 = lds[i0 + 3 * st];
+        if (DIT) {
+            Fr v = Fr::mul(x1, wc), u = Fr::mul(x3, wc);
+            x1 = Fr::sub(x0, v); x0 = Fr::add(x0, v);
+            x3 = Fr::sub(x2, u); x2 = Fr::add(x2, u);
+            v = Fr::mul(x2, wa); u = Fr::mul(x3, wb);
+            x2 = Fr::sub(x0, v); x0 = Fr::add(x0, v);
+            x3 = Fr::sub(x1, u); x1 = Fr::add(x1, u);
+        } else {
+            Fr v = Fr::sub(x0, x2), u = Fr::sub(x1, x3);
+            x0 = Fr::add(x0, x2); x1 = Fr::add(x1, x3);
+            x2 = Fr::mul(v, wa); x3 = Fr::mul(u, wb);
+            v = Fr::sub(x0, x1); u = Fr::sub(x2, x3);
+            x0 = Fr::add(x0, x1); x2 = Fr::add(x2, x3);
+            x1 = Fr::mul(v, wc); x3 = Fr::mul(u, wc);
+        }
+        lds[i0] = x0; lds[i0 + st] = x1; lds[i0 + 2 * st] = x2; lds[i0 + 3 * st] = x3;
+    }
+    __syncthreads();
+}
+template <class Fr, int DIT>
+__device__ __forceinline__ void seam_step2(Fr* lds, const Fr* __restrict__ tws, u32 l, u32 tile_elems) {
+    const Fr* t_lo = tws + ((1u << l) - 1u);
+    for (u32 q = threadIdx.x; q < (tile_elems >> 1); q += blockDim.x) {
+        u32 j = q & ((1u << l) - 1u);
+        u32 i0 = ((q >> l) << (l + 1)) | j, st = 1u << l;
+        Fr w = fr_load(&t_lo[j]);
+        Fr x0 = lds[i0], x1 = lds[i0 + st];
+        if (DIT) {
+            Fr v = Fr::mul(x1, w);
+            lds[i0] = Fr::add(x0, v);
+            lds[i0 + st] = Fr::sub(x0, v);
+        } else {
+            lds[i0] = Fr::add(x0, x1);
+            lds[i0 + st] = Fr::mul(Fr::sub(x0, x1), w);
+        }
+    }
+    __syncthreads();
+}
+template <class Fr>
+__global__ void __launch_bounds__(NTT_THREADS)
+k_ntt_seam(Fr* __restrict__ data, size_t stride_vec, const Fr* __restrict__ tw_dif, const Fr* __restrict__ tw_dit, u32 nst) {
+    extern __shared__ uint4 lds_raw[];
+    Fr* lds = reinterpret_cast<Fr*>(lds_raw);
+    const u32 tile_elems = 1u << nst;
+    Fr* vec = data + (size_t)blockIdx.y * stride_vec + ((size_t)blockIdx.x << nst);
+    for (u32 e = threadIdx.x; e < tile_elems; e += blockDim.x) lds[e] = fr_load(&vec[e]);
+    __syncthreads();
+    const u32 top = nst & ~1u;
+    if (nst > 1 && (nst & 1)) seam_step2<Fr, 0>(lds, tw_dif, nst - 1, tile_elems);
+    for (u32 l = top; l > 2; l -= 2) seam_step4<Fr, 0>(lds, tw_dif, l - 2, tile_elems);
+    if (nst == 1) {
+        if (threadIdx.x == 0) {
+            Fr x0 = lds[0], x1 = lds[1];
+            Fr v = Fr::mul(Fr::sub(x0, x1), fr_load(&tw_dit[0]));
+            x0 = Fr::add(x0, x1);
+            lds[0] = Fr::add(x0, v);
+            lds[1] = Fr::sub(x0, v);
+        }
+        __syncthreads();
+    } else {
+        const Fr w4i = fr_load(&tw_dif[2]);
+        const Fr wc = fr_load(&tw_dit[0]), wa = fr_load(&tw_dit[1]), wb = fr_load(&tw_dit[2]);
+        for (u32 q = threadIdx.x; q < (tile_elems >> 2); q += blockDim.x) {
+            u32 i0 = q << 2;
+            Fr x0 = lds[i0], x1 = lds[i0 + 1], x2 = lds[i0 + 2], x3 = lds[i0 + 3];
+            Fr v = Fr::sub(x0, x2), u = Fr::mul(Fr::sub(x1, x3), w4i);
+            x0 = Fr::add(x0, x2); x1 = Fr::add(x1, x3);
+            x2 = Fr::add(v, u); x3 = Fr::sub(v, u);
+            v = Fr::sub(x0, x1); x0 = Fr::add(x0, x1); x1 = v;
+            v = Fr::mul(x1, wc); u = Fr::mul(x3, wc);
+            x1 = Fr::sub(x0, v); x0 = Fr::add(x0, v);
+            x3 = Fr::sub(x2, u); x2 = Fr::add(x2, u);
+            v = Fr::mul(x2, wa); u = Fr::mul(x3, wb);
+            x2 = Fr::sub(x0, v); x0 = Fr::add(x0, v);
+            x3 = Fr::sub(x1, u); x1 = Fr::add(x1, u);
+            lds[i0] = x0; lds[i0 + 1] = x1; lds[i0 + 2] = x2; lds[i0 + 3] = x3;
+        }
+        __syncthreads();
+    }
+    for (u32 l = 2; l < top; l += 2) seam_step4<Fr, 1>(lds, tw_dit, l, tile_elems);
+    if (nst > 1 && (nst & 1)) seam_step2<Fr, 1>(lds, tw_dit, nst - 1, tile_elems);
+    for (u32 e = threadIdx.x; e < tile_elems; e += blockDim.x) fr_store(&vec[e], lds[e]);
+}
+
 template <class Fr>
 __global__ void k_scale_pow(Fr* __restrict__ data, size_t stride_vec, const Fr* __restrict__ pw, Fr scale,
                             u32 logn, int bitrev_index, int use_pow) {
diff --git a/hekaton_system_amd/csrc/ntt_host.cuh b/hekaton_system_amd/csrc/ntt_host.cuh
--- a/hekaton_system_amd/csrc/ntt_host.cuh
+++ b/hekaton_system_amd/csrc/ntt_host.cuh
@@ -35,6 +35,7 @@
     void* tw_inv = nullptr;
     void* pw_g = nullptr;
     void* pw_ginv = nullptr;
+    void* tw_coset[33] = {};
     std::vector<void*> retired;
 };
 
@@ -103,6 +104,35 @@
         return HK_OK;
     }
 
+    static hk_status ensure_coset(hk_ctx* ctx, u32 log_m, NttTables** out, const Fr** tco) {
+        HK_TRY(ensure(ctx, log_m, out));
+        NttTables* T = *out;
+        std::unique_lock<std::mutex> tl(T->mu);
+        *tco = (const Fr*)T->tw_coset[log_m];
+        if (*tco || log_m == 0) return HK_OK;
+        HK_HIP(hipSetDevice(ctx->device));
+        std::vector<Fr> gs(32);
+        Fr g = host_from_limbs<Fr>(C::GEN);
+        for (u32 k = 0; k < 32; k++) { gs[k] = g; g = Fr::sqr(g); }
+        Fr *d_gs = nullptr, *tab = nullptr;
+        size_t full = (size_t)1 << log_m;
+        HK_HIP(hipMalloc((void**)&d_gs, sizeof(Fr) * 32));
+        if (hipMalloc((void**)&tab, sizeof(Fr) * full) != hipSuccess) {
+            (void)hipGetLastError();
+            (void)hipFree(d_gs);
+            return HK_ERR_NOMEM;
+        }
+        HK_HIP(hipMemcpy(d_gs, gs.data(), sizeof(Fr) * 32, hipMemcpyHostToDevice));
+        hipLaunchKernelGGL((k_coset_tables<Fr>), dim3((u32)((full + 255) / 256)), dim3(256), 0, 0, tab, (const Fr*)T->tw_fwd,
+                           (const Fr*)d_gs, log_m);
+        HK_HIP(hipGetLastError());
+        HK_HIP(hipDeviceSynchronize());
+        HK_HIP(hipFree(d_gs));
+        T->tw_coset[log_m] = tab;
+        *tco = tab;
+        return HK_OK;
+    }
+
     static Fr size_inv(u32 log_m) {
         Fr x = Fr::one();
         for (u32 k = 0; k < log_m; k++) x = host_halve(x);
@@ -123,23 +153,48 @@
         const Fr* kc = nullptr;
     };
 
-    static hk_status passes(hipStream_t s, Fr* data, size_t stride, u32 batch, u32 logn, const Fr* tws, int dit,
-                            const Post& ep = Post()) {
-        if (logn == 0) return HK_OK;
-        static const u32 tile_log = [] {
+    static u32 plan_tile_log() {
+        static const u32 v = [] {
             const char* e = getenv("HK_NTT_TILE_LOG");
             return ntt_plan_tile_log(e ? (u32)atoi(e) : NTT_PLAN_TILE_LOG);
         }();
-        static const u32 upper_max = [] {
+        return v;
+    }
+    static u32 plan_upper_max() {
+        static const u32 v = [] {
             const char* e = getenv("HK_NTT_UPPER_MAX");
-            return ntt_plan_upper_max(e ? (u32)atoi(e) : NTT_PLAN_UPPER_MAX, tile_log);
+            return ntt_plan_upper_max(e ? (u32)atoi(e) : NTT_PLAN_UPPER_MAX, plan_tile_log());
         }();
+        return v;
+    }
+
+    static hk_status passes(hipStream_t s, Fr* data, size_t stride, u32 batch, u32 logn, const Fr* tws, int dit,
+                            const Post& ep = Post()) {
+        return run_plan(s, data, stride, batch, logn, tws, dit, ep, false);
+    }
+    static hk_status upper_passes(hipStream_t s, Fr* data, size_t stride, u32 batch, u32 logn, const Fr* tws, int dit) {
+        return run_plan(s, data, stride, batch, logn, tws, dit, Post(), true);
+    }
+    static hk_status seam(hipStream_t s, Fr* data, size_t stride, u32 batch, u32 logn, const Fr* tw_dif, const Fr* tw_dit) {
+        if (logn == 0) return HK_OK;
+        const u32 tile_log = plan_tile_log(), nst = logn < tile_log ? logn : tile_log;
+        hipLaunchKernelGGL((k_ntt_seam<Fr>), dim3(1u << (logn - nst), batch), dim3(1u << (tile_log - 2)), sizeof(Fr) << nst, s,
+                           data, stride, tw_dif, tw_dit, nst);
+        HK_HIP(hipGetLastError());
+        return HK_OK;
+    }
+
+    static hk_status run_plan(hipStream_t s, Fr* data, size_t stride, u32 batch, u32 logn, const Fr* tws, int dit,
+                              const Post& ep, bool upper_only) {
+        if (logn == 0) return HK_OK;
+        const u32 tile_log = plan_tile_log(), upper_max = plan_upper_max();
         const u32 threads = 1u << (tile_log - 2);
         NttPass ps[NTT_PLAN_MAX_PASSES];
         int np = ntt_pass_plan(logn, tile_log, upper_max, ps);
         Fr one = Fr::one();
         for (int k = 0; k < np; k++) {
             const NttPass& p = dit ? ps[k] : ps[np - 1 - k];
+            if (upper_only && p.lo == 0) continue;
             u32 tile_log = p.nst + p.cols_bits;
             dim3 grid(1u << (logn - tile_log), batch);
             size_t lds = sizeof(Fr) << tile_log;
@@ -251,21 +306,18 @@
         HK_HIP(hipGetLastError());
         return HK_OK;
     }
-    static hk_status run_eval(hipStream_t s, NttTables* T, const CsrDev& A, const CsrDev& B, size_t n_inst, size_t n_c,
-                              const Fr* z, Fr* ab, u32 log_m) {
+    static hk_status run_eval(hipStream_t s, NttTables* T, const Fr* tco, const CsrDev& A, const CsrDev& B, size_t n_inst,
+                              size_t n_c, const Fr* z, Fr* ab, u32 log_m) {
         size_t m = (size_t)1 << log_m;
         const CsrDev* Ms[2] = {&A, &B};
         for (int k = 0; k < 2; k++)
             hipLaunchKernelGGL((k_spmv<Fr>), dim3((u32)((m + 255) / 256)), dim3(256), 0, s,
                                Ms[k]->row_ptr, Ms[k]->col, (const Fr*)Ms[k]->val, z, ab + k * m,
                                (u32)n_c, k == 0 ? (u32)n_inst : 0u, (u32)m);
-        typename N::Post e1;
-        e1.post = 2;
-        e1.nvec = 2;
-        e1.pw = (const Fr*)T->pw_g;
-        HK_TRY(N::passes(s, ab, m, 2, log_m, (const Fr*)T->tw_inv, 0, e1));
-        HK_TRY(N::passes(s, ab, m, 2, log_m, (const Fr*)T->tw_fwd, 1));
-        hipLaunchKernelGGL((k_mul_pointwise<Fr>), dim3((u32)((m + 255) / 256)), dim3(256), 0, s, ab, ab + m, m);
+        const Fr* tinv = (const Fr*)T->tw_inv;
+        HK_TRY(N::upper_passes(s, ab, m, 2, log_m, tinv, 0));
+        HK_TRY(N::seam(s, ab, m, 2, log_m, tinv, tco));
+        HK_TRY(N::upper_passes(s, ab, m, 2, log_m, tco, 1));
         HK_HIP(hipGetLastError());
         return HK_OK;
     }
@@ -315,6 +367,8 @@
     NttTables* T = ctx->ntt;
     for (void* p : {T->tw_fwd, T->tw_inv, T->pw_g, T->pw_ginv})
         if (p) (void)hipFree(p);
+    for (void* p : T->tw_coset)
+        if (p) (void)hipFree(p);
     for (void* p : T->retired) (void)hipFree(p);
     delete T;
     ctx->ntt = nullptr;
diff --git a/hekaton_system_amd/csrc/pk.cuh b/hekaton_system_amd/csrc/pk.cuh
--- a/hekaton_system_amd/csrc/pk.cuh
+++ b/hekaton_system_amd/csrc/pk.cuh
@@ -292,7 +292,9 @@
             src = (const Affine<Fq>*)staging;
         }
         NttTables* T;
-        PK_TRY(NttHost<C>::ensure(ctx, pk->log_m, &T));
+        const Fr* tco;
+        if (pk->h_eval) PK_TRY(NttHost<C>::ensure_coset(ctx, pk->log_m, &T, &tco));
+        else PK_TRY(NttHost<C>::ensure(ctx, pk->log_m, &T));
         if (pk->h_eval) {
             PK_HIP(hipMalloc(&hb_tmp, g1 * (m + n_v)));
             Affine<Fq>*gd = (Affine<Fq>*)hb_tmp, *cd = gd + m;
@@ -320,6 +322,32 @@
 #undef PK_TRY
 
 template <class C>
+hk_status Ops<C>::pk_witness_map_eval(hk_ctx* ctx, const hk_pk* h, const void* z, size_t n_v, void* out, size_t cap) {
+    typedef QapHost<C> Q;
+    const PkImpl<C>* pk = (const PkImpl<C>*)h->impl;
+    if (h->ctx != ctx || !pk->has_qap || !pk->h_eval || !z || !out) return HK_ERR_ARG;
+    if (n_v != pk->n_v) return HK_ERR_LEN;
+    const size_t m = (size_t)1 << pk->log_m;
+    if (cap < m) return HK_ERR_LEN;
+    NttTables* T;
+    const Fr* tco;
+    HK_TRY(NttHost<C>::ensure_coset(ctx, pk->log_m, &T, &tco));
+    Staged zin = staged(z, n_v * sizeof(Fr));
+    LaneGuard g(ctx);
+    Lane* L = g.lane;
+    if (!L) return HK_ERR_DEVICE;
+    Fr* ab;
+    HK_TRY(L->carve([&](Carve& c) { stage_carve(c, &zin, 1); ab = c.n<Fr>(2 * m); }));
+    HK_TRY(stage_upload(L, &zin, 1));
+    HK_TRY(Q::run_eval(L->stream, T, tco, pk->csr[0], pk->csr[1], pk->n_inst, pk->n_c, (const Fr*)zin.p, ab, pk->log_m));
+    hipLaunchKernelGGL((k_mul_pointwise<Fr>), dim3((u32)((m + 255) / 256)), dim3(256), 0, L->stream, ab, ab + m, m);
+    HK_HIP(hipGetLastError());
+    HK_HIP(hipMemcpyAsync(out, ab, m * sizeof(Fr), is_device_ptr(out) ? hipMemcpyDeviceToDevice : hipMemcpyDeviceToHost,
+                          L->stream));
+    return L->settle();
+}
+
+template <class C>
 void Ops<C>::pk_free(hk_pk* h) {
     if (!h) return;
     PkImpl<C>* pk = (PkImpl<C>*)h->impl;
diff --git a/hekaton_system_amd/csrc/prove_impl.cuh b/hekaton_system_amd/csrc/prove_impl.cuh
--- a/hekaton_system_amd/csrc/prove_impl.cuh
+++ b/hekaton_system_amd/csrc/prove_impl.cuh
@@ -217,7 +217,9 @@
     Lane* L = g.lane;
     if (!L) return HK_ERR_DEVICE;
     NttTables* T;
-    HK_TRY(NttHost<C>::ensure(ctx, pk->log_m, &T));
+    const Fr* tco = nullptr;
+    if (pk->h_eval) HK_TRY(NttHost<C>::ensure_coset(ctx, pk->log_m, &T, &tco));
+    else HK_TRY(NttHost<C>::ensure(ctx, pk->log_m, &T));
     const MsmPlan &pz = pk->plan_z, &ph = pk->plan_h, &pa = pk->plan_a, &pb = pk->plan_b;
     const size_t m = (size_t)1 << pk->log_m, fr = sizeof(Fr), rs_stride = 2 + n_kappas;
     const size_t h_stride = (pk->h_eval ? 2 : 3) * m;
@@ -312,13 +314,14 @@
             if (prof) HK_HIP(hipEventRecord(ev[5], sH));
             for (u32 j = 0; j < nb; j++) {
                 if (pk->h_eval)
-                    HK_TRY(Q::run_eval(sH, T, pk->csr[0], pk->csr[1], pk->n_inst, pk->n_c, zd[j], abc + j * h_stride, pk->log_m));
+                    HK_TRY(Q::run_eval(sH, T, tco, pk->csr[0], pk->csr[1], pk->n_inst, pk->n_c, zd[j], abc + j * h_stride, pk->log_m));
                 else
                     HK_TRY(Q::run(sH, T, pk->csr[0], pk->csr[1], pk->csr[2], pk->n_inst, pk->n_c, zd[j],
                                   abc + j * h_stride, pk->log_m));
             }
             if (prof) HK_HIP(hipEventRecord(ev[6], sH));
-            HK_TRY(MsmSort<Fr>::run(sH, ph, (const u32*)abc, 1, sbh, true, nb, h_stride));
+            HK_TRY(MsmSort<Fr>::run(sH, ph, (const u32*)abc, 1, sbh, true, nb, h_stride,
+                                    pk->h_eval ? (const u32*)(abc + m) : nullptr));
             HK_TRY(MsmRun<Fq>::run(sH, ph, pk->h_tab, (u32)m, 0, sbh, rbh, res1 + 3, prof ? ev[12] : nullptr,
                                    prof ? ev[13] : nullptr, nb, 4));
             HK_HIP(hipEventRecord(ev[7], sH));
diff --git a/include/hekaton_testing.h b/include/hekaton_testing.h
--- /dev/null
+++ b/include/hekaton_testing.h
@@ -0,0 +1,14 @@
+#ifndef HEKATON_TESTING_H
+#define HEKATON_TESTING_H
+#include "hekaton.h"
+
+#ifdef __cplusplus
+extern "C" {
+#endif
+
+hk_status hk_pk_witness_map_eval(hk_ctx* ctx, const hk_pk* pk, const void* z_mont, size_t n_v, void* out, size_t cap);
+
+#ifdef __cplusplus
+}
+#endif
+#endif
```

Measured after the change: 137.2 (median of 6 runs). 1.4% higher.
